# FireflyRenderEngine/GPUPathTracer

Hardware: AMD Instinct MI355X
Metric: Mrays/s (path segments = closest-hit queries, device-counted) at 1080p, 8 bounces, 1024 spp (higher is better)
Workload: dtype f32; 1 GPU; C2 wahoo.obj+cube.obj Cornell box (5184 triangles, 6 planes), 1920x1080, 8 bounces, 1024 spp, camera=inside, trace=bvh, seed 1234; scene=c2, rays_per_frame=11019120206, rays_untraversed=2123366400, rays_cut_last=721266356, primary_hits_kept_between_frames=False, partition=1080-row strips round-robin over 1 rank(s), gather=none

## Files before the change

### gpupathtracer_amd/csrc/ff_api.cpp

```cpp
#include <algorithm>
#include <chrono>
#include <cmath>
#include <cstdio>
#include <cstdlib>
#include <cstring>
#include <new>
#include <vector>

#include <hip/hip_runtime.h>
#include <hip/hip_gl_interop.h>

#include "ff_state.h"

using namespace ff;

namespace {

void free_scene(FfState* s)
{
    s->primary_valid = s->last_key_valid = false;
    if (s->d_geoms) (void)hipFree(s->d_geoms);
    if (s->d_tris) (void)hipFree(s->d_tris);
    if (s->d_normals) (void)hipFree(s->d_normals);
    if (s->d_world_normals) (void)hipFree(s->d_world_normals);
// ... 72 lines not shown
    if (status == FF_OK && ue != hipSuccess) return fail(FF_ERR_HIP, "hipGraphicsUnmapResources failed: %s", hipGetErrorString(ue));
    return status;
}

}

namespace {

int check_params(const FfRenderParams* p)
{
    if (!p) return fail(FF_ERR_INVALID_ARG, "render params are null");
    if (p->width <= 0 || p->height <= 0) return fail(FF_ERR_INVALID_ARG, "image size %dx%d is invalid", p->width, p->height);
    if (p->width > 65535 || p->height > 65535) return fail(FF_ERR_INVALID_ARG, "image size %dx%d exceeds 65535 per side", p->width, p->height);
    if (p->bounces < 1 || p->bounces > 255) return fail(FF_ERR_INVALID_ARG, "bounces must be in 1..255 (got %d)", p->bounces);
    if (p->spp < 1 || p->spp >= (1 << 24)) return fail(FF_ERR_INVALID_ARG, "spp must be in 1..2^24-1 (got %d)", p->spp);
    if (p->trace_mode != FF_TRACE_BRUTE_FORCE && p->trace_mode != FF_TRACE_BVH) return fail(FF_ERR_INVALID_ARG, "unknown trace_mode %d", p->trace_mode);
    if (p->shade_mode != FF_SHADE_NORMAL_DEBUG && p->shade_mode != FF_SHADE_DIFFUSE_PATH && p->shade_mode != FF_SHADE_DIFFUSE_PATH_SMOOTH &&
        p->shade_mode != FF_SHADE_DIFFUSE_PATH_NEE) return fail(FF_ERR_INVALID_ARG, "unknown shade_mode %d", p->shade_mode);
    if (p->grid_mode != FF_GRID_FULL && p->grid_mode != FF_GRID_REFERENCE_FLOOR) return fail(FF_ERR_INVALID_ARG, "unknown grid_mode %d", p->grid_mode);
    if (p->spp_per_launch < 0) return fail(FF_ERR_INVALID_ARG, "spp_per_launch must be >= 0");
    return FF_OK;
}

}

extern "C" int ff_check_render_params(const FfRenderParams* params)
{
    clear_error();
    return check_params(params);
}

namespace ff {

int check_render_call(const FfState* s, const FfCamera* camera, const FfRenderParams* params, const char* who)
{
    if (!s) return fail(FF_ERR_INVALID_ARG, "%s: state is null", who);
    if (!camera) return fail(FF_ERR_INVALID_ARG, "%s: camera is null", who);
    const int st = check_params(params);
    if (st != FF_OK) return st;
    if (!s->has_scene) return fail(FF_ERR_NO_SCENE, "%s: no scene uploaded", who);
    return FF_OK;
}

}

namespace {

int lds_records(const FfState* s) { return s->num_geoms > kMaxLdsRecords ? 0 : s->num_geoms; }

int bvh_block_threads(const FfState* s, int preferred, int stack_levels)
{
    const int sizes[3] = { 1024, 768, 512 };
    for (int b : sizes) {
        if (b > preferred) continue;
        if (bvh_lds_bytes(0, stack_levels, b, lds_records(s)) + (s->use_pool ? pool_lds_bytes(b) : 0) <= (size_t)kLdsBudgetBytes) return b;
    }
    return 0;
}

int finalize_layout(FfState* s)
{
    int nodes4 = 0, depth4 = 0;
    for (size_t i = 0; i < s->slots.size(); ++i) {
        if (s->h_geoms[i].type != FF_GEOM_TRIANGLEMESH || s->slots[i].node4_count == 0) continue;
        nodes4 += s->slots[i].node4_count;
        depth4 = std::max(depth4, s->slots[i].depth4);
    }
    s->num_nodes4 = nodes4;
    s->max_depth4 = depth4;
    s->top_count = s->top_depth = 0;
    if (s->num_geoms > kChunkGeometries) {
        std::vector<BvhNode> top2;
        std::vector<Bvh4Node> top4;
        s->num_scan = s->sw.no_scan_planes ? 0 : count_scan_planes(s->h_geoms, s->num_quads);
        build_geometry_tree(s->h_geoms, top2, s->num_scan);
        s->top_depth = collapse_geometry_tree(top2, top4);
        s->top_count = (int)top4.size();
        if (top4.size() > (size_t)s->num_geoms) return fail(FF_ERR_HIP, "geometry tree of %zu nodes for %d geometries", top4.size(), s->num_geoms);
        FF_HIP(hipMemcpyAsync(s->d_nodes4 + s->node_capacity, top4.data(), top4.size() * sizeof(Bvh4Node), hipMemcpyHostToDevice, s->stream));
        FF_HIP(hipStreamSynchronize(s->stream));
    }
    build_wall_table(s->h_geoms.data(), s->sw.no_wall_table ? 0 : (s->num_geoms > kChunkGeometries ? s->num_scan : s->num_quads), s->walls, !s->sw.no_wall_pairs);
    if (s->num_geoms <= kChunkGeometries) add_mesh_boxes(s->h_geoms.data(), s->num_planes, s->num_geoms, s->walls);
    s->stack_entries = depth4 + 1 + (s->top_depth > 0 ? s->top_depth + 1 : 0);
    if (!s->setup_threshold_forced) {
        int biggest = 1;
        for (size_t i = 0; i < s->slots.size(); ++i) biggest = std::max(biggest, s->slots[i].node4_count);
        s->setup_threshold = std::max(4, std::min(24, (int)std::lround(1.5 * std::log((double)biggest) / std::log(4.0) - 0.7)));
        s->setup_threshold = std::min(32, s->setup_threshold + 2 * s->top_depth);
    }
    s->use_pool = s->sw.pool > 0 && s->num_geoms <= kChunkGeometries && nodes4 > 0;
    constexpr int kPoolStackLevels = 5;
    const int pool_levels = std::min(s->stack_entries, s->sw.pool_stack_levels > 0 ? s->sw.pool_stack_levels : kPoolStackLevels);
    s->scene_block_threads = bvh_block_threads(s, s->block_threads, s->use_pool ? pool_levels : s->stack_entries);
    if (s->use_pool && s->scene_block_threads != 1024) {
        s->use_pool = false;
        s->scene_block_threads = bvh_block_threads(s, s->block_threads, s->stack_entries);
    }
    const int block = s->scene_block_threads > 0 ? s->scene_block_threads : kBlockThreads;
    constexpr int kMinLdsStack = 4;
    const size_t reserve = s->use_pool ? pool_lds_bytes(block) : 0;
    s->stack_lds_levels = s->stack_entries;
    if (s->use_pool) {
        s->stack_lds_levels = pool_levels;
        while (s->stack_lds_levels < s->stack_entries && max_lds_nodes(s->stack_lds_levels + 1, block, lds_records(s), reserve) >= nodes4) ++s->stack_lds_levels;
    } else if (s->scene_block_threads > 0 && !s->sw.no_stack_spill) {
        const int want = nodes4 + s->top_count;
        if (want > max_lds_nodes(s->stack_entries, block, lds_records(s))) {
            int levels = s->stack_entries;
            while (levels > kMinLdsStack && max_lds_nodes(levels, block, lds_records(s)) < want) --levels;
            if (max_lds_nodes(levels, block, lds_records(s)) >= want) s->stack_lds_levels = levels;
        }
    }
    int cap = s->scene_block_threads > 0 ? std::max(0, max_lds_nodes(s->stack_lds_levels, block, lds_records(s), reserve)) : 0;
    if (s->sw.lds_node_cap >= 0) cap = std::min(cap, s->sw.lds_node_cap);
    s->lds_cap = std::min(cap, nodes4 + s->top_count);
    s->top_lds_count = std::min(s->top_count, cap);
    const int mesh_cap = cap - s->top_lds_count;
    constexpr int kSmallTree = 8;
    std::vector<int> share(s->h_geoms.size(), 0);
    int left = mesh_cap, wanting = 0;
    for (size_t i = 0; i < s->h_geoms.size(); ++i) {
        if (s->h_geoms[i].type != FF_GEOM_TRIANGLEMESH || s->slots[i].node4_count == 0) continue;
        share[i] = std::min(std::min(s->slots[i].node4_count, kSmallTree), left);
        left -= share[i];
        wanting += s->slots[i].node4_count - share[i];
    }
    const int pool = left;
    for (size_t i = 0; i < s->h_geoms.size() && wanting > 0; ++i) {
        if (s->h_geoms[i].type != FF_GEOM_TRIANGLEMESH || s->slots[i].node4_count == 0) continue;
        const int want = s->slots[i].node4_count - share[i];
        share[i] += wanting <= pool ? want : (int)((int64_t)pool * want / wanting);
    }
    int next = s->top_lds_count;
    for (size_t i = 0; i < s->h_geoms.size(); ++i) {
        GeomRecord& r = s->h_geoms[i];
        r.node4_first = 0;
        r.lds_nodes = 0;
        r.wmin[3] = 0.0f;
        if (r.type != FF_GEOM_TRIANGLEMESH || s->slots[i].node4_count == 0) continue;
        r.node4_first = s->slots[i].node_first;
        r.lds_nodes = std::min(s->slots[i].node4_count, share[i]);
        std::memcpy(&r.wmin[3], &next, sizeof(int));
        next += r.lds_nodes;
    }
    FF_HIP(hipMemcpyAsync(s->d_geoms, s->h_geoms.data(), s->h_geoms.size() * sizeof(GeomRecord), hipMemcpyHostToDevice, s->stream));
    if (s->d_world_normals) {
        int max_tris = 0;
        for (const GeomRecord& g : s->h_geoms) max_tris = std::max(max_tris, g.type == FF_GEOM_TRIANGLEMESH ? g.tri_count : 0);
        FF_HIP(launch_world_normals(s->d_geoms, s->d_tris, s->num_geoms, max_tris, s->d_world_normals, s->d_world_normals + s->num_tris, s->stream));
    }
    FF_HIP(hipStreamSynchronize(s->stream));
    return FF_OK;
}

int collapse_slot(FfState* s, size_t gi, bool with_info)
{
    FfState::MeshSlot& slot = s->slots[gi];
    if (slot.node_count <= 0) return FF_OK;
    int st = FF_OK;
    if (!slot.parents_linked) {
        st = gpu_link_parents(s->stream, s->d_nodes, slot.node_first, slot.node_count, s->d_parent + slot.node_first);
        if (st != FF_OK) return st;
        slot.parents_linked = true;
    }
    Collapse4Info info;
    st = gpu_collapse_mesh(s->stream, s->scratch, s->d_nodes, slot.node_first, slot.node_count, s->d_parent + slot.node_first, s->d_nodes4, slot.node_first, s->d_role + slot.node_first,
                           with_info ? &info : nullptr);
    if (st != FF_OK) return st;
    if (with_info) {
        if (info.node_count >= (1 << 22)) return fail(FF_ERR_UNSUPPORTED, "a mesh's tree has %d 4-wide nodes; the traversal stack encodes at most %d", info.node_count, (1 << 22) - 1);
        slot.node4_count = info.node_count;
        slot.depth4 = info.depth;
    }
    return FF_OK;
}

int fill_frame_mapping(const FfState* s, KParams& k, const FfCamera* camera, int W, int H, int grid_mode, int strip_rows, int part, int num_parts,
                       int local_rows, int x0, int y0, int win_w, int num_blocks, const char* who)
{
    FfMat4 cm;
    ff_camera_ray_matrix_jittered(camera, s->jitter_x, s->jitter_y, &cm);
    std::memcpy(k.cam_c0, &cm.m[0], 16);
    std::memcpy(k.cam_c1, &cm.m[4], 16);
    std::memcpy(k.cam_c2, &cm.m[8], 16);
    std::memcpy(k.cam_c3, &cm.m[12], 16);
    k.cam_pos[0] = camera->m_position.x;
    k.cam_pos[1] = camera->m_position.y;
    k.cam_pos[2] = camera->m_position.z;
    k.far_clip = camera->m_farClip;
    k.screen_w = camera->m_screenWidth;
    k.screen_h = camera->m_screenHeight;
    k.width = W;
    k.height = H;
    k.xlim = W;
    k.ylim = H;
    if (grid_mode == FF_GRID_REFERENCE_FLOOR) {
        k.xlim = (W / 16) * 16;
        k.ylim = (H / 16) * 16;
    }
    k.strip_rows = strip_rows;
    k.part = part;
    k.num_parts = num_parts;
    k.local_rows = local_rows;
    k.x0 = x0;
    k.y0 = y0;
    k.local_width = win_w;
    k.tiles_per_row = (win_w + 7) / 8;
    const uint64_t tiles = (uint64_t)k.tiles_per_row * (uint64_t)((local_rows + 7) / 8);
    if (tiles * 64 * (uint64_t)(num_blocks + 64) >= (1ull << 31)) return fail(FF_ERR_INVALID_ARG, "%simage too large for the work queue", who);
    k.pix_items = (unsigned)(tiles * 64);
    return FF_OK;
}

void fill_scene(const FfState* s, KParams& k, bool smooth, int lds_block_threads)
{
    k.setup_threshold = s->setup_threshold;
    k.leaf_threshold = s->leaf_threshold;
    k.num_geoms = s->num_geoms;
    k.num_planes = s->num_planes;
    k.num_quads = s->num_quads;
    k.has_specular = s->has_specular ? 1 : 0;
    k.geoms = s->d_geoms;
    k.tris = s->d_tris;
    k.trinormals = smooth ? reinterpret_cast<const float4*>(s->d_normals) : nullptr;
    k.nodes4 = s->d_nodes4;
    k.tri_world_normals = s->d_world_normals;
    k.geom_world_normals = s->d_world_normals ? s->d_world_normals + s->num_tris : nullptr;
    if (s->sw.lds_fill && lds_block_threads > 0) {
        const size_t bytes = bvh_lds_bytes(s->lds_cap, s->stack_lds_levels, lds_block_threads, lds_records(s));
        k.debug_lds_words = (unsigned)std::min<size_t>(s->sw.lds_fill_words, bytes / 4);
        k.debug_lds_pattern = (unsigned)s->sw.lds_fill_pattern;
    }
    k.stack_depth = s->stack_lds_levels;
    k.stack_spill = nullptr;
    k.lds_nodes = s->lds_cap;
    k.top_first = (int)s->node_capacity;
    k.top_lds_first = 0;
    k.top_lds_count = s->top_lds_count;
    k.num_scan = s->num_scan;
    k.walls = s->walls;
}

int attach_stack_spill(FfState* s, KParams& k, int grid, int block_threads)
{
    if (s->stack_lds_levels >= s->stack_entries) return FF_OK;
    const int st = ensure_bytes((void**)&s->d_stack_spill, &s->stack_spill_bytes,
                                (size_t)(s->stack_entries - s->stack_lds_levels) * (size_t)grid * (size_t)block_threads * sizeof(int));
    if (st == FF_OK) k.stack_spill = s->d_stack_spill;
    return st;
}

void size_work_queue(const FfState* s, KParams& k, int grid, int block_threads, int tail_per_wave)
{
    k.queue_counters = std::min(kQueueCountersDefault, grid);
    if (s->sw.queue_counters > 0) k.queue_counters = std::min(std::min(kQueueCounters, grid), s->sw.queue_counters);
    const int waves_per_counter = (grid * (block_threads / 64) + k.queue_counters - 1) / k.queue_counters;
    k.queue_tail_items = (unsigned)(waves_per_counter * (s->sw.queue_tail >= 0 ? s->sw.queue_tail : tail_per_wave));
}

FfState::PrimaryKey primary_key(const KParams& k, bool smooth)
{
    FfState::PrimaryKey key;
    std::memset(&key, 0, sizeof key);
    std::memcpy(key.cam, k.cam_c0, 16 * sizeof(float));
    std::memcpy(key.cam + 16, k.cam_pos, 3 * sizeof(float));
    key.cam[19] = k.far_clip; key.cam[20] = k.screen_w; key.cam[21] = k.screen_h;
    const int dims[12] = { k.width, k.height, k.xlim, k.ylim, k.strip_rows, k.part, k.num_parts, k.local_rows, k.x0, k.y0, k.local_width, smooth ? 1 : 0 };
    std::memcpy(key.dims, dims, sizeof dims);
    key.pix_items = k.pix_items;
    return key;
}

int enqueue_prepass(FfState* s, const KParams& k, float4* hits, unsigned long long* mask_out, int frame_blocks, int grid, int block_threads)
{
    KParams kp = k;
    kp.shade_mode = kShadePrimaryPass;
    kp.primary_hits = hits;
    kp.bounces = 1;
    kp.spp_total = 1;
    kp.block_spp = 1;
    kp.num_blocks = 1;
    kp.block_begin = 0;
    kp.block_end = 1;
    kp.whole_blocks = 1u;
    kp.total_items = kp.pix_items;
    kp.tail_block = -1;
    kp.cull_mask = nullptr;
    kp.cull_mask_out = mask_out;
    kp.frame_blocks = frame_blocks;
    kp.cut_last = 0;
    kp.timeline = nullptr;
    kp.queue_chunk = 32u;
    if (s->sw.queue_chunk > 0) kp.queue_chunk = (unsigned)s->sw.queue_chunk;
    FF_HIP(launch_trace(kp, FF_TRACE_BVH, false, grid, block_threads, s->stream, nullptr, false, true));
    FF_HIP(hipMemsetAsync(s->d_queue, 0, (size_t)k.queue_counters * kQueueStride * sizeof(unsigned), s->stream));
    return FF_OK;
}

}

namespace ff {

int render_enqueue(FfState* s, const FfCamera* camera, const FfRenderParams* prm, int strip_rows, int part, int num_parts, int local_rows,
                   unsigned char* rgb8_dev, float* radiance_dev, int x0, int y0, int win_w)
{
    const int W = prm->width, H = prm->height;
    if (win_w < 0) win_w = W;
    const size_t local_pixels = (size_t)local_rows * (size_t)win_w;
    s->stats = FfStats();
    s->pending = false;
    if (local_pixels == 0) return FF_OK;

    const bool debug = prm->shade_mode == FF_SHADE_NORMAL_DEBUG;
    const bool env = s->env_set && !debug;
    if (env && prm->shade_mode == FF_SHADE_DIFFUSE_PATH_SMOOTH)
        return fail(FF_ERR_UNSUPPORTED, "FF_SHADE_DIFFUSE_PATH_SMOOTH does not render under an environment light (ff_set_environment); "
                    "clear it or use FF_SHADE_DIFFUSE_PATH / FF_SHADE_DIFFUSE_PATH_NEE");
    const bool tex = s->tex_bound > 0 && !debug;
    if (tex && prm->shade_mode == FF_SHADE_DIFFUSE_PATH_SMOOTH)
        return fail(FF_ERR_UNSUPPORTED, "FF_SHADE_DIFFUSE_PATH_SMOOTH does not render albedo textures (ff_set_albedo_texture); "
                    "unbind them or use FF_SHADE_DIFFUSE_PATH / FF_SHADE_DIFFUSE_PATH_NEE");
    const bool glossy = s->glossy_applied > 0 && !debug;
    if (glossy && prm->shade_mode == FF_SHADE_DIFFUSE_PATH_SMOOTH)
// ... 139 lines not shown
        if (pst != FF_OK) return pst;
        k.park = s->d_park;
    }
    if (prm->trace_mode == FF_TRACE_BVH) {
        const int st = attach_stack_spill(s, k, grid, block_threads);
        if (st != FF_OK) return st;
    }

    {
        const int samples_per_item = std::max(1, std::min(k.block_spp, k.spp_total));
        k.queue_chunk = samples_per_item >= 64 ? (num_parts > 1 ? 32u : 64u) : (unsigned)std::min(32, std::max(4, 64 / samples_per_item));
        if (s->sw.queue_chunk > 0) k.queue_chunk = (unsigned)s->sw.queue_chunk;
        size_work_queue(s, k, grid, block_threads, samples_per_item >= 16 && !cull ? 64 : 8);
    }
    hipStream_t st = s->stream;
    if (prm->grid_mode == FF_GRID_REFERENCE_FLOOR) {
        if (rgb8_dev) FF_HIP(hipMemsetAsync(rgb8_dev, 0, local_pixels * 3, st));
        if (radiance_dev) FF_HIP(hipMemsetAsync(radiance_dev, 0, local_pixels * 3 * sizeof(float), st));
    }
    FF_HIP(hipMemsetAsync(s->d_counters, 0, (size_t)(1 + k.queue_counters) * kQueueStride * sizeof(unsigned), st));
    FF_HIP(hipEventRecord(s->ev_begin, st));
    k.tail_block = -1;
    const int last_launch_blocks = num_blocks - (launches - 1) * blocks_per_launch;
    const bool short_frame = num_parts == 1 && !s->tail_forced && num_blocks <= 8;
    const double blocks_per_lane = (double)k.pix_items * (double)last_launch_blocks / ((double)grid * (double)block_threads);
    const int tail_blocks_wanted = s->sw.tail_blocks > 0 ? s->sw.tail_blocks : (num_parts > 1 && blocks_per_lane < 24.0 ? 2 : 1);
    const int tail_blocks = std::max(1, std::min(std::min(tail_blocks_wanted, 3), last_launch_blocks - 1));
    const int tail_n = spp - (num_blocks - tail_blocks) * block_spp;
    const int tail_step = short_frame ? std::max(4, (tail_n + 3) / 4) : std::max(s->tail_group_spp * (block_spp / 64), (tail_n + 15) / 16);
    const bool tail_wanted = !debug && prm->trace_mode == FF_TRACE_BVH && s->tail_group_spp > 0 && tail_step < tail_n &&
                             (short_frame || ((num_parts > 1 || s->tail_forced) && last_launch_blocks >= s->tail_min_blocks));
    const size_t tail_bytes = (size_t)k.pix_items * (size_t)tail_n * sizeof(float4);
    const size_t tail_cap = short_frame ? std::min<size_t>(4ull << 30, s->device_mem_bytes / 50) : (16ull << 30);
    const bool tail_mode = tail_wanted && tail_bytes <= tail_cap;
    if (!tail_mode && s->d_tail_samples && s->tail_samples_bytes > (256ull << 20)) {
        (void)hipFree(s->d_tail_samples);
        s->d_tail_samples = nullptr;
        s->tail_samples_bytes = 0;
    }
    s->pending_flags = (tail_mode ? FF_STATS_TAIL_ITEMS : 0u) | (tail_wanted && !tail_mode ? FF_STATS_TAIL_SKIPPED_TOO_LARGE : 0u);
    if (tail_mode) {
        int tst = ensure_bytes((void**)&s->d_tail_samples, &s->tail_samples_bytes, tail_bytes);
        if (tst != FF_OK) return tst;
        k.tail_samples = s->d_tail_samples;
        k.tail_samples_in_block = tail_n;
        int g = 0;
        k.tail_start[0] = 0;
        while (k.tail_start[g] < tail_n && g < 16) { k.tail_start[g + 1] = std::min(tail_n, k.tail_start[g] + tail_step); ++g; }
        k.tail_groups = g;
    }
    cull = cull && num_blocks - (tail_mode ? tail_blocks : 0) > 0 && !debug;
    const bool exact_cull = reuse && !s->sw.no_primary_cull && num_blocks - (tail_mode ? tail_blocks : 0) > 0;
    const bool kept = reuse && hits_kept && (!(cull || exact_cull) || s->primary_has_mask) && start_kept;
    s->pending_mask_reused = s->pending_mask_built = false;
    if (cull || exact_cull) {
        const size_t mask_bytes = ((size_t)k.pix_items / 64 + 2) * sizeof(unsigned long long);
        if (!kept) {
            const int mst = ensure_bytes((void**)&s->d_cull_mask, &s->cull_mask_bytes, mask_bytes);
            if (mst != FF_OK) return mst;
            if (cull) FF_HIP(launch_cull_mask(k, s->d_cull_mask, st));
            else FF_HIP(hipMemsetAsync(s->d_cull_mask, 0, mask_bytes, st));
            s->pending_mask_built = true;
            if (!reuse) s->primary_has_mask = false;
        } else {
            s->pending_mask_reused = true;
        }
        k.cull_mask = s->d_cull_mask;
        s->pending_culled_rays_per_pixel = (unsigned)(spp - (tail_mode ? tail_n : 0));
    }
    if (reuse && kept) k.primary_hits = s->d_primary_cache;
    k.start_records = use_start ? s->d_start_records : nullptr;
    k.start_bounces = bounces;
    if (reuse && !kept) {
        const int pst = enqueue_prepass(s, k, s->d_primary_cache, exact_cull ? s->d_cull_mask : nullptr, num_blocks, grid, block_threads);
        if (pst != FF_OK) return pst;
        k.primary_hits = s->d_primary_cache;
        s->primary_key = key;
        s->primary_valid = true;
        s->primary_has_mask = cull || exact_cull;
        s->primary_has_start = use_start;
        s->start_bounces = bounces;
        s->start_shade = prm->shade_mode;
    }
    for (int l = 0; l < launches; ++l) {
        k.block_begin = l * blocks_per_launch;
        k.block_end = std::min(num_blocks, (l + 1) * blocks_per_launch);
        k.whole_blocks = (unsigned)(k.block_end - k.block_begin);
        k.total_items = k.pix_items * k.whole_blocks;
        if (tail_mode && l == launches - 1) {
            const unsigned groups = (unsigned)k.tail_groups;
            k.tail_block = num_blocks - tail_blocks;
            k.whole_blocks = (unsigned)(k.block_end - tail_blocks - k.block_begin);
            k.tail_first_item = k.pix_items * k.whole_blocks;
            k.total_items = k.tail_first_item + k.pix_items * groups;
        }
        if (l > 0) FF_HIP(hipMemsetAsync(s->d_queue, 0, (size_t)k.queue_counters * kQueueStride * sizeof(unsigned), st));
        FF_HIP(launch_trace(k, prm->trace_mode, s->collect_stats, grid, block_threads, st, &s->last_kernel_name, pool, false, use_start,
                            !s->sw.no_world_normals));
    }
    FF_HIP(launch_combine(k, st));
    FF_HIP(hipEventRecord(s->ev_end, st));
    FF_HIP(hipMemcpyAsync(s->h_counters, s->d_counters, kCounterWords * sizeof(unsigned long long), hipMemcpyDeviceToHost, st));
    if (k.timeline) {
        const size_t rows = (size_t)s->num_cus * 2 * (kBlockThreads / 64);
        s->h_timeline_rows.resize(rows * kTimelineBuckets);
        FF_HIP(hipMemcpyAsync(s->h_timeline_rows.data(), s->d_timeline, rows * kTimelineBuckets * sizeof(unsigned), hipMemcpyDeviceToHost, st));
    }
    s->pending = true;
    s->pending_launches = launches;
    return FF_OK;
}

int frame_primary_hits(FfState* s, const FfCamera* camera, const FfRenderParams* params, PrimaryHits* out)
{
    const int W = params->width, H = params->height;
    KParams k;
    std::memset(&k, 0, sizeof k);
    int st = fill_frame_mapping(s, k, camera, W, H, params->grid_mode, H, 0, 1, H, 0, 0, W, 1, "ff_gbuffer: ");
    if (st != FF_OK) return st;
    const size_t hits_bytes = (size_t)3 * (size_t)k.pix_items * sizeof(float4);
    bool kept = false;
    for (int smooth = 0; smooth < 2 && !kept; ++smooth) {
        const FfState::PrimaryKey key = primary_key(k, smooth != 0);
        kept = s->primary_valid && s->primary_cache_bytes >= hits_bytes && std::memcmp(&key, &s->primary_key, sizeof key) == 0;
    }
    *out = { s->d_primary_cache, !kept, k.pix_items, k.tiles_per_row, k.xlim, k.ylim };
    if (kept) return FF_OK;
    st = ensure_bytes((void**)&s->d_gb_hits, &s->gb_hits_bytes, hits_bytes);
    if (st != FF_OK) return st;
    out->hits = s->d_gb_hits;
    const int block_threads = s->scene_block_threads;
    const int grid = (int)std::max<uint64_t>(1, std::min<uint64_t>((uint64_t)s->num_cus, ((uint64_t)k.pix_items + (uint64_t)block_threads - 1) / (uint64_t)block_threads));
    fill_scene(s, k, false, block_threads);
    st = attach_stack_spill(s, k, grid, block_threads);
    if (st != FF_OK) return st;
    k.reuse_quorum = s->sw.reuse_quorum;
    k.queue = s->d_queue;
    k.counters = s->d_counters;
    k.timeline_ticks = 1;
    size_work_queue(s, k, grid, block_threads, 8);
    FF_HIP(hipMemsetAsync(s->d_counters, 0, (size_t)(1 + k.queue_counters) * kQueueStride * sizeof(unsigned), s->stream));
    return enqueue_prepass(s, k, s->d_gb_hits, nullptr, 1, grid, block_threads);
}

int render_finish(FfState* s)
{
    if (!s->pending) return FF_OK;
    s->pending = false;
    FF_HIP(hipStreamSynchronize(s->stream));
    float ms = 0.f;
    FF_HIP(hipEventElapsedTime(&ms, s->ev_begin, s->ev_end));
    unsigned long long c[32];
    std::memcpy(c, s->h_counters, sizeof c);
    std::memcpy(s->raw_counters, c, sizeof c);
    if (c[0] != 0)
        return fail(FF_ERR_HIP, "the traversal loop guard cut %llu queries short (a malformed or absurdly deep tree): the frame is not valid", c[0]);
    s->stats.rays_traced = 0;
    for (int j = 0; j < kRaySlots; ++j) s->stats.rays_traced += s->h_counters[kRaySlotStride * (kRaySlotFirst + j)];
    s->stats.rays_answered = 0;
    {
        unsigned long long culled = 0;
        for (int j = 0; j < kRaySlots; ++j) culled += s->h_counters[kCulledPixelsWord + kRaySlotStride * j];
        if (s->pending_mask_reused) culled = s->primary_culled_pixels;
        else if (s->pending_mask_built) s->primary_culled_pixels = culled;
        s->stats.rays_answered += culled * s->pending_culled_rays_per_pixel;
    }
    for (int j = 0; j < kRaySlots; ++j) s->stats.rays_answered += s->h_counters[kAnsweredWord + kRaySlotStride * j];
    s->stats.rays_cut_short = 0;
    for (int j = 0; j < kRaySlots; ++j) s->stats.rays_cut_short += s->h_counters[kCutShortWord + kRaySlotStride * j];
    s->raw_counters[0] = s->stats.rays_traced;
    s->stats.nodes_visited = c[1];
    s->stats.tris_tested = c[2];
    s->stats.planes_tested = c[3];
    s->stats.kernel_ms = ms;
    s->stats.kernel_launches = (uint32_t)s->pending_launches;
    s->stats.flags = s->pending_flags;
    s->stats.scene_bytes_nodes = (uint64_t)s->num_nodes4 * sizeof(Bvh4Node);
    s->stats.scene_bytes_tris = s->num_tris * sizeof(TriRecord);
    return FF_OK;
}

}

namespace {

int render_local(FfState* s, const FfCamera* camera, const FfRenderParams* prm, int strip_rows, int part, int num_parts, int local_rows,
                 unsigned char* rgb8_dev, float* radiance_dev, int x0 = 0, int y0 = 0, int win_w = -1)
{
    const int st = render_enqueue(s, camera, prm, strip_rows, part, num_parts, local_rows, rgb8_dev, radiance_dev, x0, y0, win_w);
    if (st != FF_OK) return st;
    return render_finish(s);
}

}

extern "C" {

namespace {
void read_switches(FfState* s)
{
    FfState::Switches w;
    w.no_last_bounce_cut = std::getenv("FF_NO_LAST_BOUNCE_CUT") != nullptr;
    w.no_primary_cull = std::getenv("FF_NO_PRIMARY_CULL") != nullptr;
    w.no_primary_reuse = std::getenv("FF_NO_PRIMARY_REUSE") != nullptr;
    w.no_primary_cache = std::getenv("FF_NO_PRIMARY_CACHE") != nullptr;
    w.no_start_records = std::getenv("FF_NO_START_RECORDS") != nullptr;
    w.no_world_normals = std::getenv("FF_NO_WORLD_NORMALS") != nullptr;
    if (const char* e = std::getenv("FF_TAIL_BLOCKS")) w.tail_blocks = std::max(1, std::min(3, std::atoi(e)));
    if (const char* e = std::getenv("FF_REUSE_MIN_SPP")) w.reuse_min_spp = std::max(1, std::atoi(e));
    if (const char* e = std::getenv("FF_REUSE_QUORUM")) w.reuse_quorum = std::max(1, std::min(65, std::atoi(e)));
    if (const char* e = std::getenv("FF_QUEUE_CHUNK")) w.queue_chunk = std::max(1, std::min(4096, std::atoi(e)));
    if (const char* e = std::getenv("FF_QUEUE_COUNTERS")) w.queue_counters = std::max(1, std::min(kQueueCounters, std::atoi(e)));
    w.no_wall_table = std::getenv("FF_NO_WALL_TABLE") != nullptr;
    w.no_wall_pairs = std::getenv("FF_NO_WALL_PAIRS") != nullptr;
    w.no_stack_spill = std::getenv("FF_NO_STACK_SPILL") != nullptr;
    w.no_scan_planes = std::getenv("FF_NO_SCAN_PLANES") != nullptr;
    if (const char* e = std::getenv("FF_DEBUG_LDS_FILL")) w.lds_fill = std::sscanf(e, "%lu,%lx", &w.lds_fill_words, &w.lds_fill_pattern) == 2;
    if (const char* e = std::getenv("FF_POOL")) w.pool = std::atoi(e) != 0 ? 1 : 0;
    if (const char* e = std::getenv("FF_POOL_QUORUM")) w.pool_quorum = std::max(1, std::min(64, std::atoi(e)));
    if (const char* e = std::getenv("FF_POOL_QUORUM_MIN")) w.pool_quorum_min = std::max(1, std::min(64, std::atoi(e)));
    if (const char* e = std::getenv("FF_POOL_REFILL")) w.pool_refill = std::max(1, std::min(64, std::atoi(e)));
    if (const char* e = std::getenv("FF_POOL_SLICE")) w.pool_slice = std::max(1, std::min(64, std::atoi(e)));
    if (const char* e = std::getenv("FF_POOL_BATCH_MIN")) w.pool_batch_min = std::max(1, std::min(1024, std::atoi(e)));
    if (const char* e = std::getenv("FF_DEBUG_LDS_NODE_CAP")) w.lds_node_cap = std::max(0, std::atoi(e));
    if (const char* e = std::getenv("FF_QUEUE_TAIL")) w.queue_tail = std::max(0, std::min(4096, std::atoi(e)));
    if (const char* e = std::getenv("FF_POOL_LEAVE")) w.pool_leave = std::max(0, std::min(64, std::atoi(e)));
    if (const char* e = std::getenv("FF_POOL_STACK_LEVELS")) w.pool_stack_levels = std::max(1, std::min(64, std::atoi(e)));
    s->sw = w;
}
}

int ff_debug_reload_switches(FfState* s)
{
    clear_error();
    if (!s) return fail(FF_ERR_INVALID_ARG, "ff_debug_reload_switches: state is null");
    read_switches(s);
    s->primary_valid = s->last_key_valid = false;
    return FF_OK;
}

int ff_create(FfState** out_state, int device_id)
{
    clear_error();
    if (!out_state) return fail(FF_ERR_INVALID_ARG, "ff_create: out_state is null");
    *out_state = nullptr;
    int count = 0;
    hipError_t e = hipGetDeviceCount(&count);
    if (e != hipSuccess || count <= 0) return fail(FF_ERR_NO_DEVICE, "ff_create: no HIP device (%s)", hipGetErrorString(e));
    if (device_id < 0 || device_id >= count) return fail(FF_ERR_INVALID_ARG, "ff_create: device %d out of range (0..%d)", device_id, count - 1);
    FF_HIP(hipSetDevice(device_id));
    hipDeviceProp_t prop;
    FF_HIP(hipGetDeviceProperties(&prop, device_id));
    FfState* s = new (std::nothrow) FfState();
    if (!s) return fail(FF_ERR_OOM, "ff_create: out of host memory");
    s->device = device_id;
    s->num_cus = prop.multiProcessorCount > 0 ? prop.multiProcessorCount : 256;
    s->device_mem_bytes = prop.totalGlobalMem;
    if (const char* bt = std::getenv("FF_BLOCK_THREADS")) {
        const int v = std::atoi(bt);
        if (v == 512 || v == 768 || v == 1024) {
            s->block_threads = v;
        }
    }
    read_switches(s);
    if (const char* e = std::getenv("FF_DEBUG_FAIL_ALLOC")) s->debug_fail_alloc = std::atoi(e);
    if (const char* e = std::getenv("FF_DEBUG_TIMELINE_US")) s->timeline_bucket_us = std::max(0, std::atoi(e));
    if (const char* e = std::getenv("FF_TAIL_MIN_BLOCKS")) s->tail_min_blocks = std::max(1, std::atoi(e));
    if (const char* e = std::getenv("FF_TAIL_GROUP")) {
        s->tail_group_spp = std::max(0, std::min(64, std::atoi(e)));
        s->tail_forced = true;
    }
    if (const char* e = std::getenv("FF_SETUP_THRESHOLD")) {
        s->setup_threshold = std::max(0, std::min(1 << 14, std::atoi(e)));
        s->setup_threshold_forced = true;
    }
    if (const char* e = std::getenv("FF_LEAF_THRESHOLD")) s->leaf_threshold = std::max(1, std::min(64, std::atoi(e)));
    hipError_t pe = prepare_kernels();
    if (pe != hipSuccess) {
        delete s;
        return fail(FF_ERR_HIP, "ff_create: kernel preparation failed: %s (is this a gfx950 device?)", hipGetErrorString(pe));
    }
    if (hipMalloc((void**)&s->d_counters, (size_t)(1 + kQueueCounters) * kQueueStride * sizeof(unsigned)) != hipSuccess ||
        hipHostMalloc((void**)&s->h_counters, kCounterWords * sizeof(unsigned long long), hipHostMallocDefault) != hipSuccess ||
        hipEventCreate(&s->ev_begin) != hipSuccess || hipEventCreate(&s->ev_end) != hipSuccess) {
        ff_destroy(s);
        return fail(FF_ERR_HIP, "ff_create: allocating work buffers failed");
    }
    s->d_queue = reinterpret_cast<unsigned*>(s->d_counters) + kQueueStride;
    *out_state = s;
    return FF_OK;
// ... 833 lines not shown
            mean_dev = s->d_mean;
        }
    }
    st = progressive_frame(s, camera, params, frame_index, rgb8_dev, mean_dev);
    if (st != FF_OK) return st;
    if (rgb8 && !rgb8_on_device) FF_HIP(hipMemcpy(rgb8, rgb8_dev, pixels * 3, hipMemcpyDeviceToHost));
    if (radiance && !radiance_on_device) FF_HIP(hipMemcpy(radiance, mean_dev, pixels * 3 * sizeof(float), hipMemcpyDeviceToHost));
    s->stats.total_ms = std::chrono::duration<double, std::milli>(std::chrono::steady_clock::now() - t0).count();
    return FF_OK;
}

int ff_render_to_pbo_progressive(FfState* s, const FfCamera* camera, const FfRenderParams* params, int frame_index)
{
    clear_error();
    const auto t0 = std::chrono::steady_clock::now();
    if (s && !s->pbo_resource) return fail(FF_ERR_GL_UNAVAILABLE, "ff_render_to_pbo_progressive: no pixel buffer registered");
    int st = check_render_call(s, camera, params, "ff_render_to_pbo_progressive");
    if (st != FF_OK) return st;
    if (params->width != s->pbo_width || params->height != s->pbo_height)
        return fail(FF_ERR_INVALID_ARG, "ff_render_to_pbo_progressive: params are %dx%d but the registered buffer is %dx%d", params->width, params->height,
                    s->pbo_width, s->pbo_height);
    FF_HIP(hipSetDevice(s->device));
    void* dptr = nullptr;
    st = map_pbo(s, (size_t)params->width * (size_t)params->height * 3, &dptr);
    if (st == FF_OK) st = unmap_pbo(s, progressive_frame(s, camera, params, frame_index, (unsigned char*)dptr, nullptr));
    s->stats.total_ms = std::chrono::duration<double, std::milli>(std::chrono::steady_clock::now() - t0).count();
    return st;
}


int ff_set_pixel_jitter(FfState* s, float jx, float jy)
{
    clear_error();
    if (!s) return fail(FF_ERR_INVALID_ARG, "ff_set_pixel_jitter: state is null");
    if (!(jx >= 0.f && jx < 1.f && jy >= 0.f && jy < 1.f))
        return fail(FF_ERR_INVALID_ARG, "ff_set_pixel_jitter: the jitter must be finite and in [0, 1) (got %g %g)", (double)jx, (double)jy);
    s->jitter_x = jx;
    s->jitter_y = jy;
    return FF_OK;
}


int ff_set_collect_stats(FfState* s, int on)
{
    clear_error();
    if (!s) return fail(FF_ERR_INVALID_ARG, "ff_set_collect_stats: state is null");
    s->collect_stats = on != 0;
    return FF_OK;
}

int ff_debug_timeline(FfState* s, unsigned* out1024, int* bucket_us)
{
    clear_error();
    if (!s || !out1024 || !bucket_us) return fail(FF_ERR_INVALID_ARG, "ff_debug_timeline: null argument");
    std::memset(s->h_timeline, 0, sizeof s->h_timeline);
    for (size_t i = 0; i < s->h_timeline_rows.size(); ++i) s->h_timeline[i % kTimelineBuckets] += s->h_timeline_rows[i];
    std::memcpy(out1024, s->h_timeline, sizeof s->h_timeline);
    *bucket_us = s->timeline_bucket_us;
    return FF_OK;
}

int ff_debug_counters(FfState* s, unsigned long long* out32)
{
    clear_error();
    if (!s || !out32) return fail(FF_ERR_INVALID_ARG, "ff_debug_counters: null argument");
    std::memcpy(out32, s->raw_counters, sizeof s->raw_counters);
    return FF_OK;
}

int ff_debug_check_ieee(FfState* s, unsigned long long* out_mismatches2)
{
    clear_error();
    if (!s || !out_mismatches2) return fail(FF_ERR_INVALID_ARG, "ff_debug_check_ieee: null argument");
    FF_HIP(hipSetDevice(s->device));
    FF_HIP(hipMemsetAsync(s->d_counters, 0, 2 * sizeof(unsigned long long), s->stream));
    FF_HIP(launch_ieee_check(s->d_counters, s->stream));
    FF_HIP(hipMemcpyAsync(out_mismatches2, s->d_counters, 2 * sizeof(unsigned long long), hipMemcpyDeviceToHost, s->stream));
    FF_HIP(hipStreamSynchronize(s->stream));
    return FF_OK;
}

const char* ff_debug_kernel_name(FfState* s) { return s && s->last_kernel_name ? s->last_kernel_name : ""; }

int ff_stats(FfState* s, FfStats* out)
{
    clear_error();
    if (!s || !out) return fail(FF_ERR_INVALID_ARG, "ff_stats: null argument");
    *out = s->stats;
    return FF_OK;
}

}
```

### gpupathtracer_amd/csrc/ff_internal.h

```cpp
#pragma once

#include <cstdarg>
#include <cstdint>
#include <string>
#include <vector>

#include "../../include/firefly/ff_api.h"
#include "ff_texture.h"

namespace ff {

int fail(int status, const char* fmt, ...) __attribute__((format(printf, 2, 3)));
void clear_error();


struct TriRecord {
    float v0[3];
    int32_t orig_index;
    float e1[3];
    float cull_margin;
    float e2[3];
    int32_t pad1;
};
static_assert(sizeof(TriRecord) == 48, "48-byte triangle record");

struct TriNormals {
    float n0[3], pad0;
    float n1[3], pad1;
    float n2[3], pad2;
};
static_assert(sizeof(TriNormals) == 48, "48-byte vertex-normal record");

struct BvhNode {
    float lmin[3];
    int32_t left;
    float lmax[3];
    int32_t right;
    float rmin[3];
    int32_t pad0;
    float rmax[3];
    int32_t pad1;
};
static_assert(sizeof(BvhNode) == 64, "64-byte BVH node");

struct Bvh4Node {
    float mn[3][4];
    float mx[3][4];
    int32_t link[4];
};
static_assert(sizeof(Bvh4Node) == 112, "112-byte 4-wide BVH node");
constexpr int32_t kEmptyLink = 0x7fffffff;

struct GeomRecord {
    float inv_c0[4], inv_c1[4], inv_c2[4], inv_c3[4];
    float mod_c0[4], mod_c1[4], mod_c2[4], mod_c3[4];
    float nrm_c0[4], nrm_c1[4], nrm_c2[4];
    float plane_n[4];
    float albedo[4];
    float emission[4];
    float wmin[4], wmax[4];
    int32_t type;
    int32_t bxdf_type;
    int32_t tri_first;
    int32_t tri_count;
    int32_t bvh_root;
    int32_t orig_index;
    int32_t node4_first;
    int32_t lds_nodes;
};
static_assert(sizeof(GeomRecord) == 16 * 16 + 32, "GeomRecord layout");

constexpr int kMaxWalls = 16;
struct Wall {
    float c;
    float cu, hu;
    float cv, hv;
    int geom;
    int hi_geom1;
    float hi_c;
};
static_assert(sizeof(Wall) == 32, "32-byte wall");
struct WallTable {
    int count[3];
    unsigned mask;
    float margin_s;
    float graze;
    int num_boxes;
    int pad;
    Wall w[kMaxWalls];
    struct MeshBox {
        float mn[3];
        int geom;
        float mx[3];
        int pad;
    } box[32];
};

void build_wall_table(const struct GeomRecord* geoms, int limit, WallTable& out, bool pairing = true);
void add_mesh_boxes(const struct GeomRecord* geoms, int first, int n, WallTable& out);

struct CompiledScene {
    std::vector<GeomRecord> geoms;
    std::vector<TriRecord> tris;
    std::vector<TriNormals> normals;
    std::vector<TriUVs> uvs;
    std::vector<BvhNode> nodes;
    int max_depth = 0;
    uint64_t total_tris = 0;
};

struct BvhBuildParams {
    int max_leaf_tris = 2;
    int device_leaf_tris = 2;
    int max_depth = 30;
    int bins = 64;
    float c_trav = 1.2f;
    int opt_passes = 1;
    int opt_max_tris = 1 << 18;
};

BvhBuildParams default_bvh_params();

int build_mesh_bvh(const FfTriangle* triangles, int count, const BvhBuildParams& params, std::vector<BvhNode>& nodes,
                   std::vector<TriRecord>& tris, int* out_depth, std::vector<TriNormals>* normals = nullptr, std::vector<TriUVs>* uvs = nullptr);

int compile_scene(const FfGeometry* geoms, int n, const BvhBuildParams& params, CompiledScene& out, bool build_bvh = true);

int build_geometry_tree(const std::vector<GeomRecord>& geoms, std::vector<BvhNode>& nodes, int first);
constexpr int kMaxScanPlanes = 8;
int count_scan_planes(const std::vector<GeomRecord>& geoms, int num_quads);

constexpr int32_t kGeomLeafBit = 0x40000000;
int collapse_geometry_tree(const std::vector<BvhNode>& binary, std::vector<Bvh4Node>& out);

void set_world_box(GeomRecord& r, const float omn[3], const float omx[3]);

}
```

### gpupathtracer_amd/csrc/ff_k_traverse.h

```cpp
#pragma once
#include "ff_k_lds.h"

namespace ff {
namespace {


constexpr int kLoopGuard = 1 << 16;
constexpr float kRel = 1.0e-4f, kAbs = 1.0e-4f;

struct Pending {
    float dist;
    int geom;
    int rec;
};

struct Segment {
    BestId best;
    Pending pend;
    unsigned meshes;
    int cur, sp, mesh;
    int tl_sp;
    int node_base;
    int lds_first, lds_count;
    int bnx, bny, bnz;
// ... 120 lines not shown
        const float sdist = tt * wlen * __builtin_amdgcn_rcpf(len);
        if (tt > 0.0f && offer(sdist, g, -1, S.pend, S.best)) {
            HitPoint H;
            resolve_pending(L, tris, wr, S.pend, S.best, H);
            offer(sdist, g, -1, S.pend, S.best);
        }
        return;
    }
    const float4 c0 = lds_geom4(L, g, 0), c1 = lds_geom4(L, g, 1), c2 = lds_geom4(L, g, 2), c3 = lds_geom4(L, g, 3);
    const float4 pn = lds_geom4(L, g, 11);
    const float ox = __builtin_fmaf(c0.x, wr.ox, __builtin_fmaf(c1.x, wr.oy, __builtin_fmaf(c2.x, wr.oz, c3.x)));
    const float oy = __builtin_fmaf(c0.y, wr.ox, __builtin_fmaf(c1.y, wr.oy, __builtin_fmaf(c2.y, wr.oz, c3.y)));
    const float oz = __builtin_fmaf(c0.z, wr.ox, __builtin_fmaf(c1.z, wr.oy, __builtin_fmaf(c2.z, wr.oz, c3.z)));
    const float ux = __builtin_fmaf(c0.x, wr.dx, __builtin_fmaf(c1.x, wr.dy, c2.x * wr.dz));
    const float uy = __builtin_fmaf(c0.y, wr.dx, __builtin_fmaf(c1.y, wr.dy, c2.y * wr.dz));
    const float uz = __builtin_fmaf(c0.z, wr.dx, __builtin_fmaf(c1.z, wr.dy, c2.z * wr.dz));
    const float nx = pn.x, ny = pn.y, nz = pn.z;
    const float dn = __builtin_fmaf(nx, ux, __builtin_fmaf(ny, uy, nz * uz));
    const float num = -__builtin_fmaf(nx, ox, __builtin_fmaf(ny, oy, nz * oz));
    const float len2 = __builtin_fmaf(ux, ux, __builtin_fmaf(uy, uy, uz * uz));
    const float q = dn * dn, qlim = 1.0e-14f * len2;
    const float ta = num * __builtin_amdgcn_rcpf(dn);
    const float Pxa = __builtin_fmaf(ta, ux, ox), Pya = __builtin_fmaf(ta, uy, oy);
    const float omag = fabsf(ox) + fabsf(oy) + fabsf(oz);
    const float delta = 1.0e-5f * (1.0f + omag) * __builtin_fmaf(fabsf(ux) + fabsf(uy), fabsf(__builtin_amdgcn_rcpf(dn)), 1.0f);
    const float ex = fabsf(Pxa), ey = fabsf(Pya);
    const bool front_sure = ta > 0.0f && fabsf(num) > 1.0e-5f * omag * (fabsf(nx) + fabsf(ny) + fabsf(nz));
    bool hit = ex <= 0.5f - delta && ey <= 0.5f - delta && front_sure && q >= qlim * 1.01f;
    float dist = ta * wlen;
    if (!hit && ex <= 0.5f + delta && ey <= 0.5f + delta && q >= qlim * 0.99f && (front_sure || fabsf(num) <= 1.0e-5f * omag * (fabsf(nx) + fabsf(ny) + fabsf(nz)))) {
        if (STATS) cnt.plane_exact += 1;
        Ray osr;
        float len;
        object_space_ray_lds(L, g, wr, osr, len);
        const float tt = plane_t(nx, ny, nz, osr);
        hit = tt > 0.0f;
        dist = tt * wlen * __builtin_amdgcn_rcpf(len);
    }
    if (hit && offer(dist, g, -1, S.pend, S.best)) {
        HitPoint H;
        resolve_pending(L, tris, wr, S.pend, S.best, H);
        offer(dist, g, -1, S.pend, S.best);
    }
}

__device__ __forceinline__ void wall_test(const Wall& w, float ixk, float oxk, float ou, float du, float ov, float dv, float dl, float tt, bool steep,
                                          float wlen, float& best_d, int& best_g, bool& tie, unsigned& slow)
{
    const float t = __builtin_fmaf(w.c, ixk, oxk);
    const float pu = __builtin_fmaf(t, du, ou), pv = __builtin_fmaf(t, dv, ov);
    const float m = fmaxf(fabsf(pu - w.cu) - w.hu, fabsf(pv - w.cv) - w.hv);
    const bool hit = m <= -dl && t > tt && steep;
    const bool miss = m > dl || t < -tt;
    slow |= (!hit && !miss) ? 1u << w.geom : 0u;
    const float d = t * wlen;
    const bool nearer = hit && best_d > __builtin_fmaf(d, 1.0f + kRel, kAbs);
    const bool farther = d > __builtin_fmaf(best_d, 1.0f + kRel, kAbs);
    tie = tie || (hit && !nearer && !farther);
    best_d = nearer ? d : best_d;
    best_g = nearer ? w.geom : best_g;
}

__device__ __forceinline__ void wall_test_pair(const Wall& w, float ixk, float oxk, float ou, float du, float ov, float dv, float dl, float tt, bool steep,
                                               float wlen, float& best_d, int& best_g, bool& tie, unsigned& slow)
{
    const float tlo = __builtin_fmaf(w.c, ixk, oxk), thi = __builtin_fmaf(w.hi_c, ixk, oxk);
    const bool up = ixk > 0.0f;
    const float t = up ? thi : tlo, tother = up ? tlo : thi;
    const int g = up ? w.hi_geom1 - 1 : w.geom, gother = up ? w.geom : w.hi_geom1 - 1;
    slow |= !(tother < -tt) ? 1u << gother : 0u;
    const float pu = __builtin_fmaf(t, du, ou), pv = __builtin_fmaf(t, dv, ov);
    const float m = fmaxf(fabsf(pu - w.cu) - w.hu, fabsf(pv - w.cv) - w.hv);
    const bool hit = m <= -dl && t > tt && steep;
    const bool miss = m > dl || t < -tt;
    slow |= (!hit && !miss) ? 1u << g : 0u;
    const float d = t * wlen;
    const bool nearer = hit && best_d > __builtin_fmaf(d, 1.0f + kRel, kAbs);
    const bool farther = d > __builtin_fmaf(best_d, 1.0f + kRel, kAbs);
    tie = tie || (hit && !nearer && !farther);
    best_d = nearer ? d : best_d;
    best_g = nearer ? g : best_g;
}

template <bool STATS>
__device__ __forceinline__ void screen_walls(const WallTable& W, const Ray& wr, const WorldSlab& ws, float wlen, Segment& S, unsigned& slow, Counters& cnt)
{
    const int nx = W.count[0], ny = nx + W.count[1], nz = ny + W.count[2];
    if (nz == 0) return;
    if (STATS) { cnt.planes += (unsigned)nz; probe_round(cnt.wall_rounds); }
    const float D = 2.0e-5f * ((fabsf(wr.ox) + fabsf(wr.oy)) + (fabsf(wr.oz) + W.margin_s));
    const float th = 0.05f * D;
    const float ax = fabsf(wr.dx), ay = fabsf(wr.dy), az = fabsf(wr.dz);
    const float aix = fabsf(ws.ix), aiy = fabsf(ws.iy), aiz = fabsf(ws.iz);
    const float gmin = W.graze * wlen;
    float best_d = kInf;
    int best_g = -1;
    bool tie = false;
    Wall cur = W.w[0];
    int i = 0;
    {
        const float dl = D * __builtin_fmaf(fmaxf(ay, az), aix, 1.0f), tt = th * aix;
        const bool steep = ax >= gmin;
        for (; i < nx; ++i) {
            const Wall nxt = W.w[min(i + 1, kMaxWalls - 1)];
            if (cur.hi_geom1) wall_test_pair(cur, ws.ix, ws.ox, wr.oy, wr.dy, wr.oz, wr.dz, dl, tt, steep, wlen, best_d, best_g, tie, slow);
            else wall_test(cur, ws.ix, ws.ox, wr.oy, wr.dy, wr.oz, wr.dz, dl, tt, steep, wlen, best_d, best_g, tie, slow);
            cur = nxt;
        }
    }
    {
        const float dl = D * __builtin_fmaf(fmaxf(az, ax), aiy, 1.0f), tt = th * aiy;
        const bool steep = ay >= gmin;
        for (; i < ny; ++i) {
            const Wall nxt = W.w[min(i + 1, kMaxWalls - 1)];
            if (cur.hi_geom1) wall_test_pair(cur, ws.iy, ws.oy, wr.oz, wr.dz, wr.ox, wr.dx, dl, tt, steep, wlen, best_d, best_g, tie, slow);
            else wall_test(cur, ws.iy, ws.oy, wr.oz, wr.dz, wr.ox, wr.dx, dl, tt, steep, wlen, best_d, best_g, tie, slow);
            cur = nxt;
        }
    }
    {
        const float dl = D * __builtin_fmaf(fmaxf(ax, ay), aiz, 1.0f), tt = th * aiz;
        const bool steep = az >= gmin;
        for (; i < nz; ++i) {
            const Wall nxt = W.w[min(i + 1, kMaxWalls - 1)];
            if (cur.hi_geom1) wall_test_pair(cur, ws.iz, ws.oz, wr.ox, wr.dx, wr.oy, wr.dy, dl, tt, steep, wlen, best_d, best_g, tie, slow);
            else wall_test(cur, ws.iz, ws.oz, wr.ox, wr.dx, wr.oy, wr.dy, dl, tt, steep, wlen, best_d, best_g, tie, slow);
            cur = nxt;
        }
    }
    if (tie) {
        slow |= W.mask;
    } else if (best_g >= 0) {
        S.pend.dist = best_d;
        S.pend.geom = best_g;
        S.pend.rec = -1;
    }
}

__device__ __forceinline__ unsigned holds(const Segment& S)
{
    return (S.pend.geom >= 0 ? 1u << (S.pend.geom & 31) : 0u) | (S.best.geom >= 0 ? 1u << (S.best.geom & 31) : 0u);
}

template <bool STATS, class LDS>
__device__ __forceinline__ bool scan_records(const LDS& L, const WallTable& W, const GeomRecord* __restrict__ geoms, int num_geoms, int num_planes,
                                           const TriRecord* __restrict__ tris, const Ray& wr, Segment& S, Counters& cnt, bool cut, unsigned emitters)
{
    const int prim_end = num_planes;
    const float wlen = __builtin_amdgcn_rcpf(inv_length(wr));

    unsigned long long tb0 = 0, tb1 = 0, tb2 = 0;
    if (STATS) tb0 = __builtin_amdgcn_s_memtime();
    const WorldSlab ws = make_world_slab(wr);
    unsigned quads = 0u;
    screen_walls<STATS>(W, wr, ws, wlen, S, quads, cnt);
    for (int g = 0; g < prim_end; ++g) {
        if ((W.mask >> g) & 1u) continue;
        const float4 bmin = lds_geom4(L, g, 14), bmax = lds_geom4(L, g, 15);
        if (slab_may_hit(bmin.x, bmin.y, bmin.z, bmax.x, bmax.y, bmax.z, ws, kInf)) quads |= 1u << g;
    }
    if (STATS) tb1 = __builtin_amdgcn_s_memtime();
    for (int guard = 0; __ballot(quads != 0u) != 0ull && guard < 32; ++guard) {
        if (quads == 0u) continue;
        const int g = __ffs((int)quads) - 1;
        quads &= quads - 1u;
        screen_analytic<STATS>(L, g, tris, wr, wlen, S, cnt);
    }

    if (STATS) tb2 = __builtin_amdgcn_s_memtime();
    S.meshes = 0u;
    const float limit = fminf(S.best.dist, S.pend.dist);
    {
        typedef unsigned box_words __attribute__((ext_vector_type(8)));
        static_assert(sizeof(WallTable::MeshBox) == 32, "one box, one load");
        box_words cur = *reinterpret_cast<const box_words*>(&W.box[0]);
        for (int i = 0; i < W.num_boxes; ++i) {
            const box_words nxt = *reinterpret_cast<const box_words*>(&W.box[min(i + 1, 31)]);
            S.meshes |= slab_may_hit(__uint_as_float(cur.s0), __uint_as_float(cur.s1), __uint_as_float(cur.s2), __uint_as_float(cur.s4), __uint_as_float(cur.s5),
                                     __uint_as_float(cur.s6), ws, limit) ? 1u << cur.s3 : 0u;
            cur = nxt;
        }
    }
    const bool over = cut && (holds(S) & emitters) == 0u;
    if (over) S.meshes = 0u;
    if (STATS && S.meshes == 0u) cnt.no_mesh += 1;
    if (STATS) {
        const unsigned long long tb3 = __builtin_amdgcn_s_memtime();
        if ((threadIdx.x & 63) == __ffsll((long long)__ballot(true)) - 1) { cnt.t_b1 += tb1 - tb0; cnt.t_b2 += tb2 - tb1; cnt.t_b3 += tb3 - tb2; }
    }
    return over;
}

template <class LDS>
__device__ __forceinline__ void enter_top(const LDS& L, const Ray& wr, Segment& S);

template <bool STATS, class LDS>
__device__ __forceinline__ void scan_walls(const LDS& L, const WallTable& W, const TriRecord* __restrict__ tris, const Ray& wr, Segment& S, Counters& cnt)
{
    const float wlen = __builtin_amdgcn_rcpf(inv_length(wr));
    const WorldSlab ws = make_world_slab(wr);
    unsigned prims = 0u;
    screen_walls<STATS>(W, wr, ws, wlen, S, prims, cnt);
    for (int g = 0; g < L.num_scan; ++g) {
        if ((W.mask >> g) & 1u) continue;
        const float4 bmin = lds_geom4(L, g, 14), bmax = lds_geom4(L, g, 15);
        if (slab_may_hit(bmin.x, bmin.y, bmin.z, bmax.x, bmax.y, bmax.z, ws, kInf)) prims |= 1u << g;
    }
    for (int guard = 0; __ballot(prims != 0u) != 0ull && guard < 8; ++guard) {
        if (prims == 0u) continue;
        const int g = __ffs((int)prims) - 1;
        prims &= prims - 1u;
        screen_analytic<STATS>(L, g, tris, wr, wlen, S, cnt);
    }
}

template <bool STATS, class LDS>
__device__ __forceinline__ bool begin_segment(const LDS& L, const WallTable& W, const GeomRecord* __restrict__ geoms, int num_geoms, int num_planes,
                                              const TriRecord* __restrict__ tris, const Ray& wr, Segment& S, Counters& cnt, bool cut = false,
                                              unsigned emitters = 0u)
{
    S.best.dist = kInf;
    S.best.geom = -1;
    S.best.rec = -1;
    S.pend.dist = kInf;
    S.pend.geom = -1;
    S.pend.rec = -1;
    S.cur = kDone;
    S.sp = 0;
    S.tl_sp = 0;
    S.mesh = -1;
    S.resume = 0;
    if constexpr (LDS::big) {
        S.meshes = 0u;
        if (L.num_scan > 0) scan_walls<STATS>(L, W, tris, wr, S, cnt);
        const bool over = cut && (holds(S) & emitters) == 0u;
        if (over) return true;
        enter_top(L, wr, S);
        S.cur = 0;
        return false;
    }
    return scan_records<STATS>(L, W, geoms, num_geoms, num_planes, tris, wr, S, cnt, cut, emitters);
}

__device__ __forceinline__ void refresh_tbound(Segment& S)
{
    S.tbound = (fminf(S.best.dist, S.pend.dist) * 1.001f + 1.0e-3f) * S.scale * 1.00001f;
}

#define FF_PIN4(q) asm volatile("" : "+v"((q).x), "+v"((q).y), "+v"((q).z), "+v"((q).w))

__device__ __forceinline__ int select_slot(const uint4 q, int c)
{
    const unsigned m0 = (unsigned)((c << 31) >> 31), m1 = (unsigned)((c << 30) >> 31);
    const unsigned lo = (q.y & m0) | (q.x & ~m0), hi = (q.w & m0) | (q.z & ~m0);
    return (int)((hi & m1) | (lo & ~m1));
}

template <class LDS>
__device__ __forceinline__ void pop_entry(const LDS& L, const uint4* __restrict__ nodes4, Segment& S, int e)
{
    if (e >= 0 && (e & kPackedEntry) != 0) {
        const int node = (e >> 8) & 0x3FFFFF;
        uint4 lk;
        if ((unsigned)node < (unsigned)S.lds_count) {
            lk = ff_smem[S.lds_first + node + 6 * L.node_cap];
            FF_PIN4(lk);
        } else {
            lk = *reinterpret_cast<const uint4*>(reinterpret_cast<const char*>(nodes4) + ((unsigned)(S.node_base + node) * (unsigned)(kNodeVec4 * 16) + 96u));
            FF_PIN4(lk);
        }
        S.cur = select_slot(lk, (e >> 2) & 3);
        const int rest = (e & 3) == 2 ? select_slot(lk, (e >> 4) & 3)
                                      : ((e & ~0xFF) | (((e >> 4) & 0xF) << 2) | 2);
        stack_push(L, S.sp - 1, rest);
    } else {
        S.cur = e;
        --S.sp;
    }
}

template <class LDS>
__device__ __forceinline__ void pop_subtree(const LDS& L, const uint4* __restrict__ nodes4, Segment& S)
{
    if (S.sp == (LDS::big ? S.tl_sp : 0)) {
        S.cur = LDS::big && S.mesh >= 0 ? kMeshDone : kDone;
        return;
    }
    pop_entry(L, nodes4, S, stack_pop(L, S.sp - 1));
}

template <class LDS>
__device__ __forceinline__ void set_box_planes(const LDS& L, Segment& S)
{
    const int q = L.node_cap * 16;
    S.bnx = S.ix < 0.0f ? 3 * q : 0;
    S.bny = S.iy < 0.0f ? 4 * q : q;
    S.bnz = S.iz < 0.0f ? 5 * q : 2 * q;
    S.bfx = 3 * q - S.bnx;
    S.bfy = 5 * q - S.bny;
    S.bfz = 7 * q - S.bnz;
}

template <class LDS>
__device__ __forceinline__ void enter_mesh(const LDS& L, int g, const Ray& wr, Segment& S)
{
    const int4 tree = lds_geom_i4(L, g, 17);
    if (tree.x < 0) return;
    float len;
    object_space_ray_lds(L, g, wr, S.osr, len);
    S.ix = safe_rcp(S.osr.dx);
    S.iy = safe_rcp(S.osr.dy);
    S.iz = safe_rcp(S.osr.dz);
    S.ox = -S.osr.ox * S.ix;
    S.oy = -S.osr.oy * S.iy;
    S.oz = -S.osr.oz * S.iz;
    set_box_planes(L, S);
    S.scale = len * inv_length(wr);
    refresh_tbound(S);
    S.mesh = g;
    S.node_base = tree.z;
    S.lds_count = tree.w;
    S.lds_first = __float_as_int(lds_geom4(L, g, 14).w);
    S.cur = 0;
    if constexpr (!LDS::big) S.sp = 0;
// ... 341 lines not shown
```

### gpupathtracer_amd/csrc/ff_kernels.h

```cpp
#pragma once

#include <hip/hip_runtime.h>

#include "ff_internal.h"

namespace ff {

constexpr int kBlockThreads = 512;
constexpr int kBlockThreadsMax = 1024;
constexpr int kLdsBudgetBytes = 160 * 1024;
constexpr int kMaxLdsRecords = 128;
constexpr int kChunkGeometries = 32;
constexpr int kBruteBatchTris = 1024;

struct KParams {
    float cam_c0[4], cam_c1[4], cam_c2[4], cam_c3[4];
    float cam_pos[3];
    float far_clip;
    float screen_w, screen_h;
    int width, height;
    int xlim, ylim;
    int strip_rows, part, num_parts, local_rows;
    int x0, y0, local_width;
    unsigned whole_blocks;
    unsigned total_items;
    unsigned queue_chunk;
    unsigned queue_tail_items;
    unsigned pix_items;
    int tiles_per_row;
    int bounces, spp_total, block_spp, block_begin, block_end, num_blocks;
    unsigned key;
    int shade_mode;
    int setup_threshold, leaf_threshold;
    int num_geoms;
    int num_planes;
    int num_quads;
    int has_specular;
    const GeomRecord* geoms;
    const TriRecord* tris;
    const float4* trinormals;
    int num_scan;
    const Bvh4Node* nodes4;
    int top_first, top_lds_first, top_lds_count;
    int lds_nodes;
    int stack_depth;
    int* stack_spill;
    float4* blocksums;
    unsigned char* rgb8;
    float* radiance;
    unsigned* queue;
    int queue_counters;
    int tail_block;
    int tail_groups;
    int tail_start[17];
    int tail_samples_in_block;
    unsigned tail_first_item;
    float4* tail_samples;
    unsigned long long* counters;
    unsigned debug_lds_words, debug_lds_pattern;
    const unsigned long long* cull_mask;
    unsigned long long* cull_mask_out;
    int frame_blocks;
    float4* primary_hits;
    int reuse_quorum;
    unsigned emitter_mask;
    int cut_last;
    float scene_min[3], scene_max[3];
    WallTable walls;
    float4* park;
    int pool_quorum, pool_quorum_min, pool_refill, pool_slice, pool_leave, pool_batch_min;
    unsigned* timeline;
    unsigned timeline_ticks;
    float4* start_records;
    int start_bounces;
    const float4* tri_world_normals;
    const float4* geom_world_normals;
};
constexpr int kRaySlots = 30, kRaySlotFirst = 2, kRaySlotStride = 16;
constexpr int kAnsweredWord = kRaySlotStride * kRaySlotFirst + 1;
constexpr int kCutShortWord = kRaySlotStride * kRaySlotFirst + 3;
constexpr int kCulledPixelsWord = kRaySlotStride * kRaySlotFirst + 2;
constexpr int kCounterWords = 512;
constexpr int kTimelineBuckets = 1024;
constexpr int kQueueCounters = 64;
constexpr int kQueueCountersDefault = 16;
constexpr int kQueueStride = 1024;
constexpr int kShadePrimaryPass = 100;
constexpr int kQueueStripe = 64;
constexpr int kQueueTailWord = 64;

struct RayBatchParams {
    const FfRay* rays;
    FfIntersect* out;
    int n;
    int num_geoms;
    int num_planes;
    int num_quads;
    const GeomRecord* geoms;
    const TriRecord* tris;
    const Bvh4Node* nodes4;
    int top_first, top_lds_first, top_lds_count;
    int lds_nodes;
    int stack_depth;
    int* stack_spill;
    int num_scan;
    WallTable walls;
    unsigned long long* guard_hits;
};

constexpr unsigned kNeeKeySelect = 0x6A09E667u;
constexpr unsigned kNeeKeyPoint = 0xBB67AE85u;
struct NeeParams {
    KParams k;
    const float4* lights;
    int num_lights;
    const float* light_pdf;
    unsigned items;
    const float4* env_texels;
    const float2* env_alias;
    const float* env_z;
    int env_w, env_h;
    float env_rotation;
    float p_env;
    float p_area;
    const TexBinding* tex_bind;
    const TexDesc* tex_desc;
    const TriUVs* uvs;
    const float* glossy_alpha;
    int cam_active, cam_box;
    float cam_lens_radius, cam_focus;
    float cam_fwd[3], cam_right[3], cam_up[3];
};
constexpr unsigned kEnvKeyChoose = 0x3C6EF372u;
constexpr unsigned kCameraKeyPixel = 0xA54FF53Au;
constexpr unsigned kCameraKeyLens = 0x510E527Fu;

size_t bvh_lds_bytes(int lds_nodes, int stack_depth, int block_threads, int num_geoms);
int max_lds_nodes(int stack_depth, int block_threads, int num_geoms, size_t reserve = 0);
size_t pool_lds_bytes(int block_threads);

hipError_t launch_trace(const KParams& p, int trace_mode, bool collect_stats, int grid_blocks, int block_threads, hipStream_t stream,
                        const char** kernel_name = nullptr, bool pool = false, bool prepass = false, bool start = false, bool world_normals = false);
hipError_t launch_world_normals(const GeomRecord* geoms, const TriRecord* tris, int num_geoms, int max_tri_count, float4* tri_out, float4* geom_out,
                                hipStream_t stream);
hipError_t launch_combine(const KParams& p, hipStream_t stream);
hipError_t launch_cull_mask(const KParams& p, unsigned long long* mask, hipStream_t stream);
hipError_t launch_accumulate(float* sum, const float* frame, float* mean, unsigned char* rgb8, size_t values, int first_frame, float inv_frames,
                             hipStream_t stream);
hipError_t launch_ray_batch(const RayBatchParams& p, int trace_mode, hipStream_t stream);
hipError_t launch_ieee_check(unsigned long long* mismatches2, hipStream_t stream);
hipError_t launch_deinterleave(const void* src, void* dst, int width, int height, int strip_rows, int num_parts, int elem_bytes,
                               hipStream_t stream);
hipError_t launch_unpack_strips(const void* src, unsigned char* rgb8, float* radiance, int width, int height, int strip_rows, int num_parts,
                                hipStream_t stream);
hipError_t launch_nee(const NeeParams& np, int trace_mode, bool env, bool tex, bool glossy, int grid_blocks, hipStream_t stream, const char** kernel_name);
hipError_t prepare_kernels();

}
```

### gpupathtracer_amd/csrc/ff_kernels.hip

```cpp
#include "ff_k_traverse.h"
#include "ff_k_shade.h"

namespace ff {
namespace {


template <bool STATS, int BLOCK, bool EXTRAS, int BIG = 0, bool PREPASS = false, bool START = false, bool WN = false>
__global__ __launch_bounds__(BLOCK) void trace_bvh_kernel(const KParams p)
{
    static_assert(!START || (!EXTRAS && BIG == 0 && !PREPASS), "start records: the diffuse small-scene kernel only");
    static_assert(!WN || (!EXTRAS && BIG == 0 && !PREPASS), "normal tables: the diffuse small-scene kernels only");
    const int tid = threadIdx.x;
    const int lane = tid & (kWave - 1);
    const LdsT<BIG> L = make_lds<BIG>(p.lds_nodes, p.stack_depth, BLOCK, tid, EXTRAS ? p.num_quads : 0x7fffffff, EXTRAS ? p.trinormals : nullptr,
                                      p.geoms, p.top_first, p.top_lds_first, p.top_lds_count, BIG ? p.num_scan : 0, p.stack_spill);
    const uint4* nodes4 = reinterpret_cast<const uint4*>(p.nodes4);
    if (p.debug_lds_words != 0u) {
        for (unsigned i = tid; i < p.debug_lds_words; i += BLOCK) reinterpret_cast<unsigned*>(ff_smem)[i] = p.debug_lds_pattern;
        __syncthreads();
    }
    stage_scene(L, nodes4, p.geoms, p.num_geoms, p.num_planes, tid, BLOCK);
    if constexpr (WN) {
        for (int g = tid; g < p.num_planes; g += BLOCK) reinterpret_cast<float4*>(ff_smem)[L.geom_base + g * kGeomVec4 + kGeomWorldNormalVec4] = p.geom_world_normals[g];
        __syncthreads();
    }

    Counters cnt = {};
    Path P;
    init_path(P);
    WaveQueue Q = make_wave_queue(p);
    Segment S;
    S.best = { kInf, -1, -1 };
    S.pend = { kInf, -1, -1 };
    S.meshes = 0u;
    S.cur = kDone; S.sp = 0; S.mesh = -1; S.resume = 0;
    S.osr = { 0.f, 0.f, 0.f, 0.f, 0.f, 1.f };
    S.ix = S.iy = S.iz = S.ox = S.oy = S.oz = 0.f;
    S.scale = 1.f;
    S.tbound = 0.f;
    S.node_base = 0; S.lds_first = 0; S.lds_count = 0; S.tl_sp = 0;
    S.bnx = S.bny = S.bnz = S.bfx = S.bfy = S.bfz = 0;
    bool active = false, exhausted = false, inflight = false;
    const bool reuse = START || (!PREPASS && p.primary_hits != nullptr);
    auto stored_hit = [&](int k) { return p.primary_hits + (size_t)k * p.pix_items + ((unsigned)P.item & kItemPixelMask); };
    unsigned long long tphase[5] = { 0, 0, 0, 0, 0 };
    const unsigned long long wave_t0 = STATS ? wall_clock64() : 0ull;
    unsigned long long epoch = 0ull;
    if (STATS && p.timeline) {
        if (lane == 0) {
            const unsigned long long seen = atomicCAS(&p.counters[27], 0ull, wave_t0);
            epoch = seen ? seen : wave_t0;
        }
        epoch = __shfl(epoch, 0);
    }
    unsigned* const tl_row = STATS && p.timeline ? p.timeline + (size_t)(blockIdx.x * (BLOCK / kWave) + tid / kWave) * kTimelineBuckets : nullptr;
    int tl_bucket = 0;
    unsigned tl_count = 0u;
    for (;;) {
        unsigned long long t0 = 0, t1 = 0, t2 = 0, t3 = 0, t4 = 0;
        if (STATS) t0 = __builtin_amdgcn_s_memtime();
        const bool setup = !inflight || segment_done(S);
        if (STATS && p.timeline) {
            const int finished = __popcll(__ballot(setup && inflight));
            if (finished) {
                const unsigned long long now = wall_clock64();
                const unsigned long long bb = now > epoch ? (now - epoch) / p.timeline_ticks : 0ull;
                const int b = bb < (unsigned long long)kTimelineBuckets ? (int)bb : kTimelineBuckets - 1;
                if (b != tl_bucket) {
                    if (lane == 0 && tl_count) tl_row[tl_bucket] += tl_count;
                    tl_bucket = b;
                    tl_count = 0u;
                }
                tl_count += (unsigned)finished;
            }
        }
        Best best;
        bool hit = false;
        bool shade_now = setup && inflight;
        if (shade_now) {
            finish_segment<WN>(L, p.tris, P.ray, S, best, p.tri_world_normals);
            hit = best.geom >= 0;
        }
        if (STATS) t1 = __builtin_amdgcn_s_memtime();
        if constexpr (START) {
            bool from_rec = setup && !inflight && active && P.b == 0;
            bool goes_on = false;
            MaterialRef M;
            M.global = nullptr;
            M.geom_base = L.geom_base;
            M.g = 0;
            if (shade_now) {
                M.g = best.geom;
                const int r = settle_hit<false, false, WN>(p, best, hit, M, P);
                inflight = false;
// ... 4 lines not shown
            float4 q0 = make_float4(0.f, 0.f, 0.f, 0.f), q1 = q0;
            if (from_rec) {
                const float4* rec = p.start_records + ((unsigned)P.item & kItemPixelMask);
                q0 = rec[0];
                q1 = rec[p.pix_items];
                cnt.rays += 1;
                goes_on = true;
            }
            {
                const unsigned reused_now = (unsigned)__popcll(__ballot(from_rec));
                cnt.reused += reused_now;
                if (STATS && p.timeline) tl_count += reused_now;
            }
            if (goes_on) scatter_start<WN>(p, best, M, P, from_rec, q0, q1);
        } else {
            bool from_cache = setup && !inflight && active && P.b == 0 && reuse;
            bool settle_now = shade_now, goes_on = false;
            for (;;) {
                if (from_cache) {
                    const float4 c0 = *stored_hit(0), c1 = *stored_hit(1), c2 = *stored_hit(2);
                    best.dist = c0.x; best.px = c0.y; best.py = c0.z; best.pz = c0.w;
                    best.cx = c1.x; best.cy = c1.y; best.cz = c1.z;
                    best.geom = __float_as_int(c1.w);
                    best.rec = __float_as_int(c2.x);
                    hit = best.geom >= 0;
                    if constexpr (WN) {
                        float4 n = make_float4(0.f, 0.f, 1.f, 0.f);
                        if (hit) {
                            if (best.rec >= 0) n = p.tri_world_normals[best.rec];
                            else n = lds_geom4(L, best.geom, kGeomWorldNormalVec4);
                        }
                        best.cx = n.x; best.cy = n.y; best.cz = n.z;
                    }
                    cnt.rays += 1;
                    settle_now = true;
                }
                {
                    const unsigned reused_now = (unsigned)__popcll(__ballot(from_cache));
                    cnt.reused += reused_now;
                    if (STATS && p.timeline) tl_count += reused_now;
                }
                if (__ballot(settle_now) == 0ull) break;
                bool waiting = false;
                if (settle_now) {
                    MaterialRef M;
                    M.global = BIG == 2 ? p.geoms + (hit ? best.geom : 0) : nullptr;
                    M.geom_base = L.geom_base;
                    M.g = best.geom;
                    const int r = settle_hit<EXTRAS, PREPASS, WN>(p, best, hit, M, P);
                    inflight = false;
                    active = r != kPixelDone;
                    goes_on = r == kGoesOn;
                    waiting = r == kNewSample && reuse;
                }
                settle_now = false;
                from_cache = waiting && __popcll(__ballot(waiting)) >= p.reuse_quorum;
            }
            if (goes_on) {
                MaterialRef M;
                M.global = BIG == 2 ? p.geoms + best.geom : nullptr;
                M.geom_base = L.geom_base;
                M.g = best.geom;
                scatter<EXTRAS, WN>(p, best, M, P);
            }
        }
        if (STATS) t2 = __builtin_amdgcn_s_memtime();
        {
            const bool need = setup && !active && !exhausted;
            if (__ballot(need) != 0ull) {
                const unsigned rays_before = cnt.rays;
                const bool got = acquire_pixel<START>(p, lane, P, Q, need, cnt.rays, &cnt.reused);
                if (STATS && p.timeline) tl_count += (unsigned)wave_sum((unsigned long long)(cnt.rays - rays_before));
                if (need) {
                    active = got;
                    exhausted = !got;
                    if (STATS && exhausted) atomicMax(&p.counters[23], ~(unsigned long long)wall_clock64());
                }
            }
        }
        if (STATS) t3 = __builtin_amdgcn_s_memtime();
        bool over = false;
        if (setup && active && !(P.b == 0 && reuse)) {
            if (STATS) probe_round(cnt.segment_rounds);
            over = begin_segment<STATS>(L, p.walls, p.geoms, p.num_geoms, p.num_planes, p.tris, P.ray, S, cnt, p.cut_last != 0 && P.b == p.bounces - 1, p.emitter_mask);
            cnt.rays += 1;
            inflight = true;
        }
        cnt.cut += (unsigned)__popcll(__ballot(over));
        if (STATS) t4 = __builtin_amdgcn_s_memtime();
        if (__ballot(inflight || (active && P.b == 0 && reuse)) == 0ull) break;
        if (inflight) traverse_budget<STATS>(L, p.tris, nodes4, P.ray, S, cnt, p.setup_threshold, p.leaf_threshold, p.num_planes);
        if (STATS) {
            const unsigned long long t5 = __builtin_amdgcn_s_memtime();
            tphase[0] += t1 - t0; tphase[1] += t2 - t1; tphase[2] += t3 - t2; tphase[3] += t4 - t3; tphase[4] += t5 - t4;
        }
    }
    if (STATS && p.timeline && lane == 0 && tl_count) tl_row[tl_bucket] += tl_count;
    if (STATS && lane == 0) {
        atomicAdd(&p.counters[4], tphase[0]);
        atomicAdd(&p.counters[5], tphase[1]);
        atomicAdd(&p.counters[6], tphase[2]);
        atomicAdd(&p.counters[7], tphase[3]);
        atomicAdd(&p.counters[13], tphase[4]);
        atomicMax(&p.counters[22], tphase[0] + tphase[1] + tphase[2] + tphase[3] + tphase[4]);
        atomicMax(&p.counters[24], ~(unsigned long long)wave_t0);
        atomicMax(&p.counters[25], (unsigned long long)wall_clock64());
    }
    flush_counters(p, lane, cnt, STATS);
}


constexpr int kPoolRing = 2048;
constexpr unsigned kRingEmpty = 0xFFFFu;
constexpr int kPoolSpinLimit = 1 << 20;
constexpr int kPendEmpty = -2;
constexpr int kPendOwner = -3;
constexpr unsigned kJobReturned = 0x80000000u;
constexpr unsigned kJobTie = 0x40000000u;

struct PoolOccupancy {
    unsigned inner_rounds, inner_lanes;
    unsigned leaf_rounds, leaf_lanes;
};

struct PoolRef {
    int job_base;
    int ring_base;
    int ctrl;
};

__device__ __forceinline__ unsigned* pool_u32() { return reinterpret_cast<unsigned*>(ff_smem); }
__device__ __forceinline__ unsigned short* pool_u16() { return reinterpret_cast<unsigned short*>(ff_smem); }

__device__ __forceinline__ void pool_push(const PoolRef& Q, int lane, int slot, bool post)
{
    const unsigned long long m = __ballot(post);
    if (m == 0ull) return;
    __builtin_amdgcn_fence(__ATOMIC_RELEASE, "workgroup");
    const int leader = __ffsll((long long)m) - 1;
    unsigned base = 0u;
    if (lane == leader) base = __hip_atomic_fetch_add(&pool_u32()[Q.ctrl + 1], (unsigned)__popcll(m), __ATOMIC_RELAXED, __HIP_MEMORY_SCOPE_WORKGROUP);
    base = (unsigned)__builtin_amdgcn_readlane((int)base, leader);
    if (post) {
        const unsigned rank = (unsigned)__popcll(m & ((1ull << lane) - 1ull));
        __hip_atomic_store(&pool_u16()[Q.ring_base + (int)((base + rank) & (unsigned)(kPoolRing - 1))], (unsigned short)slot, __ATOMIC_RELAXED, __HIP_MEMORY_SCOPE_WORKGROUP);
    }
}

__device__ __forceinline__ int pool_pop(const PoolRef& Q, int lane, bool want, bool& stuck)
{
    const unsigned long long m = __ballot(want);
    const unsigned asked = (unsigned)__popcll(m);
    unsigned h = 0u, n = 0u;
    if (lane == 0) {
        for (int tries = 0; tries < kPoolSpinLimit; ++tries) {
            h = __hip_atomic_load(&pool_u32()[Q.ctrl], __ATOMIC_RELAXED, __HIP_MEMORY_SCOPE_WORKGROUP);
            const unsigned t = __hip_atomic_load(&pool_u32()[Q.ctrl + 1], __ATOMIC_RELAXED, __HIP_MEMORY_SCOPE_WORKGROUP);
            n = min(asked, t - h);
            if (n == 0u) break;
            unsigned expect = h;
            if (__hip_atomic_compare_exchange_strong(&pool_u32()[Q.ctrl], &expect, h + n, __ATOMIC_RELAXED, __ATOMIC_RELAXED, __HIP_MEMORY_SCOPE_WORKGROUP)) break;
            n = 0u;
        }
    }
    h = (unsigned)__builtin_amdgcn_readfirstlane((int)h);
    n = (unsigned)__builtin_amdgcn_readfirstlane((int)n);
    int slot = -1;
// ... 545 lines not shown
    if (live) {
        const FfRay r = p.rays[i];
        wr.ox = r.m_origin.x; wr.oy = r.m_origin.y; wr.oz = r.m_origin.z;
        wr.dx = r.m_direction.x; wr.dy = r.m_direction.y; wr.dz = r.m_direction.z;
    }
    Best best;
    best.dist = kInf; best.geom = -1; best.rec = -1; best.px = best.py = best.pz = 0.f; best.cx = best.cy = 0.f; best.cz = 1.f;
    Counters cnt = {};
    if (MODE == FF_TRACE_BRUTE_FORCE) closest_hit_brute<false>(p.geoms, p.num_geoms, p.tris, batch, live, wr, best, cnt);
    else if (live) closest_hit_deferred<false>(L, p.walls, p.geoms, p.num_geoms, p.num_planes, p.tris, nodes4, wr, best, cnt);
    if (live && ((cnt.guard_hits >> (threadIdx.x & 63)) & 1ull) != 0ull && p.guard_hits) atomicAdd(p.guard_hits, 1ull);
    if (!live) return;
    FfIntersect out;
    out.m_intersectionPoint.x = 0.f; out.m_intersectionPoint.y = 0.f; out.m_intersectionPoint.z = 0.f;
    out.m_normal.x = 0.f; out.m_normal.y = 0.f; out.m_normal.z = 0.f;
    out.m_t = 0.f;
    out.m_hit = 0;
    out._pad[0] = out._pad[1] = out._pad[2] = 0;
    out.geometryIndex = -1;
    out.triangleIndex = -1;
    if (best.geom >= 0) {
        const GeomRecord& G = p.geoms[best.geom];
        MaterialRef M;
        M.global = &G;
        M.geom_base = L.geom_base;
        M.g = 0;
        float nx, ny, nz;
        world_normal(M, best, true, nx, ny, nz);
        out.m_intersectionPoint.x = best.px; out.m_intersectionPoint.y = best.py; out.m_intersectionPoint.z = best.pz;
        out.m_normal.x = nx; out.m_normal.y = ny; out.m_normal.z = nz;
        out.m_t = best.dist;
        out.m_hit = 1;
        out.geometryIndex = G.orig_index;
        out.triangleIndex = best.rec >= 0 ? p.tris[best.rec].orig_index : -1;
    }
    p.out[i] = out;
}

}
}

#include "ff_k_nee.h"

namespace ff {

#if defined(FF_PROBE) || defined(FF_PROBE_NEE)
namespace {
#ifdef FF_PROBE
template __global__ void FF_PROBE(const KParams);
#else
template __global__ void FF_PROBE_NEE(const NeeParams);
#endif
}
#else
size_t bvh_lds_bytes(int lds_nodes, int stack_depth, int block_threads, int num_geoms)
{
    return (size_t)lds_nodes * sizeof(Bvh4Node) + (size_t)stack_depth * (size_t)block_threads * sizeof(unsigned) +
           (size_t)num_geoms * sizeof(GeomRecord);
}

int max_lds_nodes(int stack_depth, int block_threads, int num_geoms, size_t reserve)
{
    const long avail = (long)kLdsBudgetBytes - (long)reserve - (long)stack_depth * (long)block_threads * (long)sizeof(unsigned) -
                       (long)num_geoms * (long)sizeof(GeomRecord);
    return avail > 0 ? (int)(avail / (long)sizeof(Bvh4Node)) : 0;
}

static int scene_size_class(int num_geoms) { return num_geoms <= kChunkGeometries ? 0 : (num_geoms <= kMaxLdsRecords ? 1 : 2); }

static size_t trace_lds_bytes(bool bvh, int lds_nodes, int stack_depth, int block_threads, int num_geoms, int big)
{
    return bvh ? bvh_lds_bytes(lds_nodes, stack_depth, block_threads, big == 2 ? 0 : num_geoms) : (size_t)kBruteBatchTris * sizeof(TriRecord);
}

static bool needs_extras(const KParams& p) { return p.num_planes > p.num_quads || p.has_specular != 0 || p.trinormals != nullptr; }

template <class K>
static hipError_t allow_full_lds(K* kernel)
{
    return hipFuncSetAttribute(reinterpret_cast<const void*>(kernel), hipFuncAttributeMaxDynamicSharedMemorySize, kLdsBudgetBytes);
}


#define FF_TRACE_BVH_KERNELS_OF(X, B)                                                                                                                \
    X(false, B, false, 0, false, false, false) X(true, B, false, 0, false, false, false) X(false, B, true, 0, false, false, false)                   \
    X(true, B, true, 0, false, false, false) X(false, B, true, 1, false, false, false) X(true, B, true, 1, false, false, false)                      \
    X(false, B, true, 2, false, false, false) X(true, B, true, 2, false, false, false)                                                               \
    X(false, B, true, 0, true, false, false) X(false, B, true, 1, true, false, false) X(false, B, true, 2, true, false, false)                       \
    X(false, B, false, 0, false, true, false) X(true, B, false, 0, false, true, false)                                                               \
    X(false, B, false, 0, false, false, true) X(true, B, false, 0, false, false, true)                                                               \
    X(false, B, false, 0, false, true, true) X(true, B, false, 0, false, true, true)
#define FF_TRACE_BVH_KERNELS(X) FF_TRACE_BVH_KERNELS_OF(X, 512) FF_TRACE_BVH_KERNELS_OF(X, 768) FF_TRACE_BVH_KERNELS_OF(X, 1024)
#define FF_NAME_START_false ""
#define FF_NAME_START_true ", true"
#define FF_RAY_BATCH_KERNELS(X) X(FF_TRACE_BVH, 0) X(FF_TRACE_BVH, 1) X(FF_TRACE_BVH, 2) X(FF_TRACE_BRUTE_FORCE, 0)

#define FF_TRACE_POOL_KERNELS(X) X(false, 1024, false) X(false, 1024, true) X(true, 1024, false) X(true, 1024, true)

#define FF_NEE_KERNELS_OF(X, MODE, BIG)                                                                               \
    X(MODE, BIG, 0, 0, 0, 0, "")           X(MODE, BIG, 1, 0, 0, 0, ", 1")                                            \
    X(MODE, BIG, 0, 1, 0, 0, ", 0, 1")     X(MODE, BIG, 1, 1, 0, 0, ", 1, 1")                                         \
    X(MODE, BIG, 0, 0, 1, 0, ", 0, 0, 1")  X(MODE, BIG, 1, 0, 1, 0, ", 1, 0, 1")                                      \
    X(MODE, BIG, 0, 1, 1, 0, ", 0, 1, 1")  X(MODE, BIG, 1, 1, 1, 0, ", 1, 1, 1")                                      \
    X(MODE, BIG, 0, 0, 0, 1, ", 0, 0, 0, 1") X(MODE, BIG, 1, 0, 0, 1, ", 1, 0, 0, 1")                                 \
    X(MODE, BIG, 0, 1, 0, 1, ", 0, 1, 0, 1") X(MODE, BIG, 1, 1, 0, 1, ", 1, 1, 0, 1")                                 \
    X(MODE, BIG, 0, 0, 1, 1, ", 0, 0, 1, 1") X(MODE, BIG, 1, 0, 1, 1, ", 1, 0, 1, 1")                                 \
    X(MODE, BIG, 0, 1, 1, 1, ", 0, 1, 1, 1") X(MODE, BIG, 1, 1, 1, 1, ", 1, 1, 1, 1")
#define FF_NEE_KERNELS(X) FF_NEE_KERNELS_OF(X, 1, 0) FF_NEE_KERNELS_OF(X, 1, 1) FF_NEE_KERNELS_OF(X, 1, 2) FF_NEE_KERNELS_OF(X, 0, 0)
static_assert(FF_TRACE_BVH == 1 && FF_TRACE_BRUTE_FORCE == 0, "the MODE column and the reported names spell the trace modes as numerals");

hipError_t prepare_kernels()
{
    hipError_t e;
#define FF_X(STATS, B, EXTRAS, BIG, PREPASS, START, WN) \
    if ((e = allow_full_lds(&trace_bvh_kernel<STATS, B, EXTRAS, BIG, PREPASS, START, WN>)) != hipSuccess) return e;
    FF_TRACE_BVH_KERNELS(FF_X)
#undef FF_X
#define FF_X(STATS, B, EXTRAS) \
    if ((e = allow_full_lds(&trace_pool_kernel<STATS, B, EXTRAS>)) != hipSuccess) return e;
    FF_TRACE_POOL_KERNELS(FF_X)
#undef FF_X
#define FF_X(MODE, BIG) \
    if (MODE == FF_TRACE_BVH && (e = allow_full_lds(&ray_batch_kernel<MODE, BIG>)) != hipSuccess) return e;
    FF_RAY_BATCH_KERNELS(FF_X)
#undef FF_X
#define FF_X(MODE, BIG, ENV, TEX, GLOSSY, CAM, TAIL) \
    if (MODE == FF_TRACE_BVH && (e = allow_full_lds(&nee_path_kernel<MODE, BIG, ENV, TEX, GLOSSY, CAM>)) != hipSuccess) return e;
    FF_NEE_KERNELS(FF_X)
#undef FF_X
    return hipSuccess;
}

size_t pool_lds_bytes(int block_threads) { return (size_t)block_threads * 48 + (size_t)kPoolRing * 2 + 128; }

static hipError_t launch_pool(const KParams& p, bool collect_stats, int grid_blocks, int block_threads, hipStream_t stream, const char** kernel_name)
{
    const dim3 grid(grid_blocks), block(block_threads);
    const size_t lds = bvh_lds_bytes(p.lds_nodes, p.stack_depth, block_threads, p.num_geoms) + pool_lds_bytes(block_threads);
    const bool extras = needs_extras(p);
    const char* name = "";
#define FF_X(STATS, B, EXTRAS)                                                                                  \
    if (collect_stats == STATS && block_threads == B && extras == EXTRAS) {                                     \
        hipLaunchKernelGGL((trace_pool_kernel<STATS, B, EXTRAS>), grid, block, lds, stream, p);                 \
        name = "trace_pool_kernel<" #STATS ", " #B ", " #EXTRAS ">";                                            \
    } else
    FF_TRACE_POOL_KERNELS(FF_X) return hipErrorInvalidValue;
#undef FF_X
    if (kernel_name) *kernel_name = name;
    return hipGetLastError();
}

hipError_t launch_trace(const KParams& p, int trace_mode, bool collect_stats, int grid_blocks, int block_threads, hipStream_t stream,
                        const char** kernel_name, bool pool, bool prepass, bool start, bool world_normals)
{
    const dim3 grid(grid_blocks);
    const char* name = "";
    if (!prepass && trace_mode == FF_TRACE_BVH && pool && p.num_geoms <= kChunkGeometries && block_threads == 1024)
        return launch_pool(p, collect_stats, grid_blocks, block_threads, stream, kernel_name);
    if (prepass || trace_mode == FF_TRACE_BVH) {
        const dim3 block(block_threads);
        const int big = scene_size_class(p.num_geoms);
        const size_t lds = trace_lds_bytes(true, p.lds_nodes, p.stack_depth, block_threads, p.num_geoms, big);
        if (!prepass && start && (big != 0 || needs_extras(p) || p.start_records == nullptr)) return hipErrorInvalidValue;
        const int threads = block_threads == 1024 ? 1024 : (block_threads == 768 ? 768 : 512);
        const bool stats = !prepass && collect_stats, extras = prepass || big != 0 || needs_extras(p), from_start = !prepass && start;
        const bool wn = world_normals && !extras && p.shade_mode == FF_SHADE_DIFFUSE_PATH && p.tri_world_normals != nullptr && p.geom_world_normals != nullptr;
#define FF_X(STATS, B, EXTRAS, BIG, PREPASS, START, WN)                                                                                              \
    if (stats == STATS && threads == B && extras == EXTRAS && big == BIG && prepass == PREPASS && from_start == START && wn == WN) {                 \
        hipLaunchKernelGGL((trace_bvh_kernel<STATS, B, EXTRAS, BIG, PREPASS, START, WN>), grid, block, lds, stream, p);                              \
        name = "trace_bvh_kernel<" #STATS ", " #B ", " #EXTRAS ", " #BIG ", " #PREPASS FF_NAME_START_##START ">";                                    \
    } else
        FF_TRACE_BVH_KERNELS(FF_X) return hipErrorInvalidValue;
#undef FF_X
        if (prepass) name = "trace_bvh_kernel<false, B, true, big, true>";
    } else {
        const size_t lds = (size_t)kBruteBatchTris * sizeof(TriRecord);
        const dim3 block(kBlockThreads);
        if (collect_stats) hipLaunchKernelGGL((trace_brute_kernel<true>), grid, block, lds, stream, p);
        else hipLaunchKernelGGL((trace_brute_kernel<false>), grid, block, lds, stream, p);
        name = collect_stats ? "trace_brute_kernel<true>" : "trace_brute_kernel<false>";
    }
    if (kernel_name) *kernel_name = name;
    return hipGetLastError();
}

hipError_t launch_ray_batch(const RayBatchParams& p, int trace_mode, hipStream_t stream)
{
    if (p.n <= 0) return hipSuccess;
    const bool bvh = trace_mode == FF_TRACE_BVH;
    const int mode = bvh ? FF_TRACE_BVH : FF_TRACE_BRUTE_FORCE, big = scene_size_class(p.num_geoms), big_key = bvh ? big : 0;
    const size_t lds = trace_lds_bytes(bvh, p.lds_nodes, p.stack_depth, kBlockThreads, p.num_geoms, big);
    const dim3 grid((p.n + kBlockThreads - 1) / kBlockThreads), block(kBlockThreads);
#define FF_X(MODE, BIG) \
    if (mode == MODE && big_key == BIG) hipLaunchKernelGGL((ray_batch_kernel<MODE, BIG>), grid, block, lds, stream, p); else
    FF_RAY_BATCH_KERNELS(FF_X) return hipErrorInvalidValue;
#undef FF_X
    return hipGetLastError();
}

hipError_t launch_nee(const NeeParams& np, int trace_mode, bool env, bool tex, bool glossy, int grid_blocks, hipStream_t stream, const char** kernel_name)
{
    if (np.items == 0u) return hipSuccess;
    const KParams& p = np.k;
    const bool bvh = trace_mode == FF_TRACE_BVH, cam = np.cam_active != 0;
    const int mode = bvh ? 1 : 0, big = scene_size_class(p.num_geoms), big_key = bvh ? big : 0;
    const size_t lds = trace_lds_bytes(bvh, p.lds_nodes, p.stack_depth, kBlockThreads, p.num_geoms, big);
    const dim3 grid(grid_blocks), block(kBlockThreads);
    const char* name = "";
#define FF_X(MODE, BIG, ENV, TEX, GLOSSY, CAM, TAIL)                                                                  \
    if (mode == MODE && big_key == BIG && env == (ENV != 0) && tex == (TEX != 0) && glossy == (GLOSSY != 0) && cam == (CAM != 0)) { \
        hipLaunchKernelGGL((nee_path_kernel<MODE, BIG, ENV, TEX, GLOSSY, CAM>), grid, block, lds, stream, np);        \
        name = "nee_path_kernel<" #MODE ", " #BIG TAIL ">";                                                           \
    } else
    FF_NEE_KERNELS(FF_X) return hipErrorInvalidValue;
#undef FF_X
    if (kernel_name) *kernel_name = name;
    return hipGetLastError();
}

#endif
}
```

### gpupathtracer_amd/csrc/ff_scene.cpp

```cpp
#include <algorithm>
#include <atomic>
#include <cfloat>
#include <cmath>
#include <cstdio>
#include <cstdlib>
#include <cstring>
#include <limits>
#include <numeric>
#include <queue>
#include <system_error>
#include <thread>

#include "ff_internal.h"
#include "ff_math.h"

namespace ff {

namespace {

struct Box {
    float mn[3], mx[3];
    void reset()
    {
        for (int k = 0; k < 3; ++k) {
// ... 601 lines not shown
        for (int k = 0; k < 3; ++k) { mn[k] = std::min(mn[k], r.wmin[k]); mx[k] = std::max(mx[k], r.wmax[k]); }
    }
    const double scene = box_half_area(mn, mx);
    int n = 0;
    while (n < num_quads && n < kMaxScanPlanes && n + 2 < (int)geoms.size() && scene > 0.0 && box_half_area(geoms[n].wmin, geoms[n].wmax) >= 0.08 * scene) ++n;
    return n;
}

void build_wall_table(const GeomRecord* geoms, int limit, WallTable& out, bool pairing)
{
    std::memset(&out, 0, sizeof out);
    struct Found {
        int axis;
        Wall w;
    };
    std::vector<Found> found;
    float scale_s = 0.f, ratio = 1.f;
    for (int g = 0; g < limit && g < 32 && (int)found.size() < kMaxWalls; ++g) {
        const GeomRecord& r = geoms[g];
        if (r.type != FF_GEOM_PLANE) continue;
        if (!(r.plane_n[0] == 0.f && r.plane_n[1] == 0.f && r.plane_n[2] == 1.f)) continue;
        const float* col[3] = { r.mod_c0, r.mod_c1, r.mod_c2 };
        int dom[3];
        float len[3];
        bool ok = true;
        for (int j = 0; j < 3 && ok; ++j) {
            const float a0 = std::fabs(col[j][0]), a1 = std::fabs(col[j][1]), a2 = std::fabs(col[j][2]);
            dom[j] = a0 >= a1 && a0 >= a2 ? 0 : (a1 >= a2 ? 1 : 2);
            len[j] = std::sqrt(a0 * a0 + a1 * a1 + a2 * a2);
            if (!(len[j] > 1e-20f && len[j] < 1e20f)) ok = false;
            for (int k = 0; k < 3 && ok; ++k)
                if (k != dom[j] && std::fabs(col[j][k]) > 2.0e-7f * len[j]) ok = false;
        }
        if (!ok || dom[0] == dom[1] || dom[0] == dom[2] || dom[1] == dom[2]) continue;
        const float smax = std::max(len[0], std::max(len[1], len[2])), smin = std::min(len[0], std::min(len[1], len[2]));
        if (!(smax <= 16.f * smin)) continue;
        const float* T = r.mod_c3;
        if (!(std::fabs(T[0]) < 1e8f && std::fabs(T[1]) < 1e8f && std::fabs(T[2]) < 1e8f)) continue;
        Found f;
        f.axis = dom[2];
        const int u = (f.axis + 1) % 3, v = (f.axis + 2) % 3;
        const float hu = 0.5f * (dom[0] == u ? len[0] : len[1]), hv = 0.5f * (dom[0] == v ? len[0] : len[1]);
        std::memset(&f.w, 0, sizeof f.w);
        f.w.c = T[f.axis];
        f.w.cu = T[u];
        f.w.hu = hu;
        f.w.cv = T[v];
        f.w.hv = hv;
        f.w.geom = g;
        found.push_back(f);
        ratio = std::max(ratio, smax / smin);
        scale_s = std::max(scale_s, smax + std::fabs(T[0]) + std::fabs(T[1]) + std::fabs(T[2]));
    }
    std::vector<char> used(found.size(), 0);
    int n = 0;
    for (int axis = 0; axis < 3; ++axis)
        for (size_t i = 0; i < found.size(); ++i) {
            if (found[i].axis != axis || used[i]) continue;
            used[i] = 1;
            Wall w = found[i].w;
            out.mask |= 1u << w.geom;
            for (size_t j = i + 1; pairing && j < found.size(); ++j) {
                const Wall& o = found[j].w;
                if (found[j].axis != axis || used[j] || o.c == w.c) continue;
                if (std::memcmp(&o.cu, &w.cu, 4 * sizeof(float)) != 0) continue;
                used[j] = 1;
                out.mask |= 1u << o.geom;
                const Wall& lo = o.c < w.c ? o : w;
                const Wall& hi = o.c < w.c ? w : o;
                Wall both = lo;
                both.hi_geom1 = hi.geom + 1;
                both.hi_c = hi.c;
                w = both;
                break;
            }
            out.w[n++] = w;
            out.count[axis] += 1;
        }
    out.margin_s = ratio * scale_s;
    out.graze = 1.2e-7f * ratio;
    if (ratio > 1.f) {
        out.margin_s += (ratio - 1.f) * 3.f * scale_s;
    }
}

void add_mesh_boxes(const GeomRecord* geoms, int first, int n, WallTable& out)
{
    out.num_boxes = 0;
    for (int g = first; g < n && g < 32; ++g) {
        const GeomRecord& r = geoms[g];
        if (r.type != FF_GEOM_TRIANGLEMESH || r.bvh_root < 0) continue;
        WallTable::MeshBox& b = out.box[out.num_boxes++];
        for (int k = 0; k < 3; ++k) { b.mn[k] = r.wmin[k]; b.mx[k] = r.wmax[k]; }
        b.geom = g;
        b.pad = 0;
    }
}

int collapse_geometry_tree(const std::vector<BvhNode>& binary, std::vector<Bvh4Node>& out)
{
    out.clear();
    if (binary.empty()) return 0;
    std::vector<int> order(1, 0), index4(binary.size(), -1), level(1, 1);
    index4[0] = 0;
    auto grandchildren = [&](int n, int links[4], const float* mn[4], const float* mx[4]) {
        int slots = 0;
        const BvhNode& nd = binary[n];
        for (int side = 0; side < 2; ++side) {
            const int link = side == 0 ? nd.left : nd.right;
            if (link < 0) {
                links[slots] = link; mn[slots] = side == 0 ? nd.lmin : nd.rmin; mx[slots] = side == 0 ? nd.lmax : nd.rmax; ++slots;
            } else {
                const BvhNode& ch = binary[link];
                links[slots] = ch.left; mn[slots] = ch.lmin; mx[slots] = ch.lmax; ++slots;
                links[slots] = ch.right; mn[slots] = ch.rmin; mx[slots] = ch.rmax; ++slots;
            }
        }
        return slots;
    };
    int depth = 1;
    for (size_t i = 0; i < order.size(); ++i) {
        int links[4];
        const float *mn[4], *mx[4];
        const int slots = grandchildren(order[i], links, mn, mx);
        for (int q = 0; q < slots; ++q)
            if (links[q] >= 0) {
                index4[links[q]] = (int)order.size();
                order.push_back(links[q]);
                level.push_back(level[i] + 1);
                depth = std::max(depth, level[i] + 1);
            }
    }
    out.resize(order.size());
    for (size_t i = 0; i < order.size(); ++i) {
        int links[4];
        const float *mn[4], *mx[4];
        const int slots = grandchildren(order[i], links, mn, mx);
        Bvh4Node& o = out[i];
        for (int q = 0; q < 4; ++q) {
            for (int k = 0; k < 3; ++k) {
                o.mn[k][q] = q < slots ? mn[q][k] : std::numeric_limits<float>::infinity();
                o.mx[k][q] = q < slots ? mx[q][k] : -std::numeric_limits<float>::infinity();
            }
            o.link[q] = q >= slots ? kEmptyLink : (links[q] >= 0 ? index4[links[q]] : ~(kGeomLeafBit | ~links[q]));
        }
    }
    return depth;
}

void set_world_box(GeomRecord& r, const float omn[3], const float omx[3])
{
    using namespace ffm;
    M4 mod;
    mod.c[0] = v4(r.mod_c0[0], r.mod_c0[1], r.mod_c0[2], 0.f);
    mod.c[1] = v4(r.mod_c1[0], r.mod_c1[1], r.mod_c1[2], 0.f);
    mod.c[2] = v4(r.mod_c2[0], r.mod_c2[1], r.mod_c2[2], 0.f);
    mod.c[3] = v4(r.mod_c3[0], r.mod_c3[1], r.mod_c3[2], 1.f);
    Box wb;
    wb.reset();
    if (omn[0] <= omx[0]) {
        for (int c = 0; c < 8; ++c) {
            const V4 pw = mul(mod, v4((c & 1) ? omx[0] : omn[0], (c & 2) ? omx[1] : omn[1], (c & 4) ? omx[2] : omn[2], 1.f));
            wb.grow(&pw.x);
        }
        float big = 0.f;
        for (int k = 0; k < 3; ++k) big = std::max(big, std::max(std::fabs(wb.mn[k]), std::fabs(wb.mx[k])) + (wb.mx[k] - wb.mn[k]));
// ... 163 lines not shown

}
}

extern "C" int ff_scene_info(const FfGeometry* host_geometries, int n, FfSceneInfo* out)
{
    using namespace ff;
    clear_error();
    if (!out) return fail(FF_ERR_INVALID_ARG, "ff_scene_info: out_info is null");
    std::memset(out, 0, sizeof *out);
    CompiledScene cs;
    const BvhBuildParams bp = default_bvh_params();
    const int st = compile_scene(host_geometries, n, bp, cs);
    if (st != FF_OK) return st;
    out->num_geometries = (int)cs.geoms.size();
    for (const GeomRecord& g : cs.geoms) {
        if (g.type == FF_GEOM_TRIANGLEMESH) ++out->num_meshes;
        else ++out->num_planes;
    }
    out->bvh_nodes = (int)cs.nodes.size();
    out->bvh_max_depth = cs.max_depth;
    out->num_triangles = cs.tris.size();
    const int stack_depth = cs.max_depth + 1;
    out->lds_nodes = std::min((int)cs.nodes.size(), std::max(0, max_lds_nodes(stack_depth, 512, (int)cs.geoms.size())));
    out->lds_bytes = (int)bvh_lds_bytes(out->lds_nodes, stack_depth, 512, (int)cs.geoms.size());
    out->device_bytes = cs.geoms.size() * sizeof(GeomRecord) + cs.tris.size() * sizeof(TriRecord) + cs.nodes.size() * sizeof(BvhNode);
    int max_leaf = 0;
    out->valid = check_bvh(cs, &max_leaf) ? 1 : 0;
    out->bvh_max_leaf = max_leaf;
    double area = 0.0;
    for (const BvhNode& nd : cs.nodes) {
        const float* lo[2] = { nd.lmin, nd.rmin };
        const float* hi[2] = { nd.lmax, nd.rmax };
        for (int c = 0; c < 2; ++c) {
            const double dx = (double)hi[c][0] - lo[c][0], dy = (double)hi[c][1] - lo[c][1], dz = (double)hi[c][2] - lo[c][2];
            if (dx >= 0.0 && dy >= 0.0 && dz >= 0.0) area += dx * dy + dy * dz + dz * dx;
        }
    }
    out->bvh_child_area = (float)area;
    return FF_OK;
}

extern "C" int ff_debug_wall_table(const FfGeometry* host_geometries, int n, float* out_walls7, int max_walls)
{
    using namespace ff;
    clear_error();
    CompiledScene cs;
    const int st = compile_scene(host_geometries, n, default_bvh_params(), cs, false);
    if (st != FF_OK) return -st;
    int num_quads = 0;
    for (const GeomRecord& g : cs.geoms) num_quads += g.type == FF_GEOM_PLANE ? 1 : 0;
    WallTable t;
    build_wall_table(cs.geoms.data(), num_quads, t, std::getenv("FF_NO_WALL_PAIRS") == nullptr);
    int count = 0, i = 0;
    for (int axis = 0; axis < 3; ++axis)
        for (int k = 0; k < t.count[axis]; ++k, ++i) {
            const Wall& w = t.w[i];
            for (int side = 0; side < (w.hi_geom1 ? 2 : 1); ++side) {
                if (out_walls7 && count < max_walls) {
                    float* o = out_walls7 + (size_t)count * 7;
                    o[0] = (float)cs.geoms[side ? w.hi_geom1 - 1 : w.geom].orig_index;
                    o[1] = (float)axis;
                    o[2] = side ? w.hi_c : w.c; o[3] = w.cu; o[4] = w.hu; o[5] = w.cv; o[6] = w.hv;
                }
                ++count;
            }
        }
    return count;
}

extern "C" int ff_debug_wall_entries(const FfGeometry* host_geometries, int n)
{
    using namespace ff;
    clear_error();
    CompiledScene cs;
    const int st = compile_scene(host_geometries, n, default_bvh_params(), cs, false);
    if (st != FF_OK) return -st;
    int num_quads = 0;
    for (const GeomRecord& g : cs.geoms) num_quads += g.type == FF_GEOM_PLANE ? 1 : 0;
    WallTable t;
    build_wall_table(cs.geoms.data(), num_quads, t, std::getenv("FF_NO_WALL_PAIRS") == nullptr);
    return t.count[0] + t.count[1] + t.count[2];
}
```

### gpupathtracer_amd/csrc/ff_state.h

```cpp
#pragma once

#include <vector>

#include <hip/hip_runtime.h>

#include "ff_build.h"
#include "ff_image.h"
#include "ff_internal.h"
#include "ff_kernels.h"
#include "ff_texture.h"

struct FfDistContext;

struct FfState {
    int device = 0;
    int num_cus = 0;
    size_t device_mem_bytes = 0;
    hipStream_t stream = nullptr;
    ff::GeomRecord* d_geoms = nullptr;
    ff::TriRecord* d_tris = nullptr;
    ff::TriNormals* d_normals = nullptr;
    ff::TriUVs* d_uvs = nullptr;
    float4* d_world_normals = nullptr;
    ff::BvhNode* d_nodes = nullptr;
    ff::WallTable walls = {};
    int num_scan = 0;
    ff::Bvh4Node* d_nodes4 = nullptr;
    int num_geoms = 0, num_planes = 0, num_quads = 0, num_nodes = 0, max_depth = 0;
    int num_nodes4 = 0, max_depth4 = 0;
    int top_count = 0, top_depth = 0, top_lds_count = 0;
    int stack_entries = 1;
    int stack_lds_levels = 1;
    unsigned long long* d_cull_mask = nullptr;
    size_t cull_mask_bytes = 0;
    float4* d_primary_cache = nullptr;
    size_t primary_cache_bytes = 0;
    float4* d_start_records = nullptr;
    size_t start_records_bytes = 0;
    bool primary_has_start = false;
    int start_bounces = 0, start_shade = 0;
    struct PrimaryKey {
        float cam[24];
        int dims[12];
        unsigned pix_items;
    } primary_key = {};
    bool primary_valid = false;
    PrimaryKey last_key = {};
    bool last_key_valid = false;
    bool primary_has_mask = false;
    unsigned long long primary_culled_pixels = 0;
    bool pending_mask_reused = false, pending_mask_built = false;
    float4* d_park = nullptr;
    size_t park_bytes = 0;
    int* d_stack_spill = nullptr;
    size_t stack_spill_bytes = 0;
    bool use_pool = false;
    int scene_block_threads = 0, lds_cap = 0;
    bool has_specular = false;
    uint64_t num_tris = 0;
    bool has_scene = false;
    struct MeshSlot {
        int node_first = 0, node_count = 0, node_capacity = 0, depth = 0;
        int node4_count = 0, depth4 = 0;
        bool parents_linked = false;
    };
    int builder = FF_BUILD_HOST_SAH;
    int scene_builder = FF_BUILD_HOST_SAH;
    std::vector<ff::GeomRecord> h_geoms;
    std::vector<MeshSlot> slots;
    size_t node_capacity = 0;
    int* d_parent = nullptr;
    unsigned char* d_role = nullptr;
    FfTriangle* d_stage = nullptr;
    size_t stage_bytes = 0;
    ff::BuildScratch scratch;
    FfBuildStats build_stats = {};
    float* d_blocksums = nullptr;
    size_t blocksums_bytes = 0;
    unsigned char* d_rgb8 = nullptr;
    size_t rgb8_bytes = 0;
    float* d_radiance = nullptr;
    size_t radiance_bytes = 0;
    float4* d_tail_samples = nullptr;
    size_t tail_samples_bytes = 0;
    bool tail_forced = false;
    int tail_min_blocks = 4;
    int tail_group_spp = 8;
    float* d_accum = nullptr;
    size_t accum_bytes = 0;
    float* d_frame = nullptr;
    size_t frame_bytes = 0;
    float* d_mean = nullptr;
    size_t mean_bytes = 0;
    int accum_width = 0, accum_height = 0, accum_frames = 0;
    float4* d_gb_hits = nullptr;
    size_t gb_hits_bytes = 0;
    void* d_img_stage = nullptr;
    size_t img_stage_bytes = 0;
    float4* d_dn_work = nullptr;
    size_t dn_work_bytes = 0;
    enum { kHistoryTemporal = 0, kHistoryTaa = 1, kHistoryTaaUpscale = 2 };
    ff::ReprojectionHistory history[3];
    int taa_upscale_lo_width = 0, taa_upscale_lo_height = 0;
    float jitter_x = 0.f, jitter_y = 0.f;
    FfCameraSampling cam_sampling = { FF_PIXEL_CORNER, 0.f, 1.f, 0 };
    bool cam_active() const { return cam_sampling.pixel_filter == FF_PIXEL_BOX || cam_sampling.lens_radius > 0.f; }
    std::vector<FfGeometry> nee_geoms;
    std::vector<FfBXDF> nee_bxdfs;
    std::vector<std::vector<FfTriangle>> nee_tris;
    bool nee_valid = false;
    int nee_num_lights = 0;
    float4* d_nee_lights = nullptr;
    size_t nee_lights_bytes = 0;
    float* d_nee_pdf = nullptr;
    size_t nee_pdf_bytes = 0;
    bool env_set = false;
    bool env_sampled = false;
    int env_w = 0, env_h = 0;
    float env_rotation = 0.f;
    float4* d_env_texels = nullptr;
    size_t env_texels_bytes = 0;
    float2* d_env_alias = nullptr;
    size_t env_alias_bytes = 0;
    float* d_env_z = nullptr;
    size_t env_z_bytes = 0;
    struct Texture {
        float4* d_texels = nullptr;
        int w = 0, h = 0, flags = 0;
    };
    std::vector<Texture> textures;
    std::vector<ff::TexBinding> tex_bindings;
    int tex_bound = 0;
    ff::TexBinding* d_tex_bind = nullptr;
    size_t tex_bind_bytes = 0;
    ff::TexDesc* d_tex_desc = nullptr;
    size_t tex_desc_bytes = 0;
    std::vector<float> glossy_roughness;
    int glossy_applied = 0;
    float* d_glossy_alpha = nullptr;
    size_t glossy_alpha_bytes = 0;
    void* d_disp_const = nullptr;
    size_t disp_const_bytes = 0;
    void* d_disp_work = nullptr;
    size_t disp_work_bytes = 0;
    bool disp_has_prev = false, disp_called = false;
    float disp_prev_exposure = 0.f;
    float disp_exposure = 0.f, disp_target = 0.f;
    uint32_t disp_histogram[256] = {};
    void* d_mblur_work = nullptr;
    size_t mblur_work_bytes = 0;
    void* d_dof_work = nullptr;
    size_t dof_work_bytes = 0;
    void* d_despeckle_work = nullptr;
    size_t despeckle_work_bytes = 0;
    unsigned* d_queue = nullptr;
    unsigned long long* d_counters = nullptr;
    unsigned long long* h_counters = nullptr;
    hipEvent_t ev_begin = nullptr, ev_end = nullptr;
    bool collect_stats = false;
    struct Switches {
        bool no_last_bounce_cut = false, no_primary_cull = false, no_primary_reuse = false;
        bool no_start_records = false;
        bool no_world_normals = false;
        bool no_primary_cache = false;
        int tail_blocks = 0;
        int reuse_min_spp = 2;
        int reuse_quorum = 1;
        int queue_chunk = 0, queue_counters = 0;
        int queue_tail = -1;
        bool no_wall_table = false, no_wall_pairs = false, no_stack_spill = false, no_scan_planes = false;
        bool lds_fill = false;
        unsigned long lds_fill_words = 0, lds_fill_pattern = 0;
        int pool = -1;
        int pool_quorum = 0;
        int pool_quorum_min = 0;
        int pool_refill = 0;
        int pool_slice = 0;
        int pool_batch_min = 0;
        int lds_node_cap = -1;
        int pool_leave = -1;
        int pool_stack_levels = 0;
    } sw;
    int block_threads = ff::kBlockThreadsMax;
    bool setup_threshold_forced = false;
    int setup_threshold = 14, leaf_threshold = 20;
    FfStats stats;
    const char* last_kernel_name = nullptr;
    unsigned long long raw_counters[32] = {};
    hipGraphicsResource* pbo_resource = nullptr;
    int pbo_width = 0, pbo_height = 0;
    FfDistContext* dist = nullptr;
    int pending_launches = 0;
    uint32_t pending_flags = 0;
    unsigned pending_culled_rays_per_pixel = 0;
    bool pending = false;
    int debug_fail_alloc = -1, alloc_countdown = -1;
    int timeline_bucket_us = 0;
    unsigned* d_timeline = nullptr;
    unsigned h_timeline[1024] = {};
    std::vector<unsigned> h_timeline_rows;
};


#define FF_HIP(call)                                                                                          \
    do {                                                                                                      \
        hipError_t _e = (call);                                                                               \
        if (_e != hipSuccess) return fail(_e == hipErrorOutOfMemory ? FF_ERR_OOM : FF_ERR_HIP, "%s failed: %s (%s:%d)", #call, hipGetErrorString(_e), __FILE__, __LINE__); \
    } while (0)

namespace ff {

int ensure_bytes(void** ptr, size_t* cap, size_t need);

int check_render_call(const FfState* s, const FfCamera* camera, const FfRenderParams* params, const char* who);

int render_enqueue(FfState* s, const FfCamera* camera, const FfRenderParams* prm, int strip_rows, int part, int num_parts, int local_rows,
                   unsigned char* rgb8_dev, float* radiance_dev, int x0 = 0, int y0 = 0, int win_w = -1);
int render_finish(FfState* s);

struct PrimaryHits {
    const float4* hits;
    bool fresh;
    unsigned pix_items;
    int tiles_per_row, xlim, ylim;
};
int frame_primary_hits(FfState* s, const FfCamera* camera, const FfRenderParams* params, PrimaryHits* out);

void dist_release(FfState* s);

void nee_capture(FfState* s, const FfGeometry* g, int n, bool upload);
void nee_replace_mesh(FfState* s, int geometry_index, const FfTriangle* tris, int count);
int nee_rebuild(FfState* s);
int enqueue_nee(FfState* s, KParams& k, const FfCamera* camera, const FfRenderParams* prm, int launches, int blocks_per_launch, size_t local_pixels);
int check_camera_sampling(const FfCameraSampling* cs, const char* who);
void env_release(FfState* s);
void tex_drop_bindings(FfState* s);
int tex_sync_tables(FfState* s);
void tex_release(FfState* s);
void glossy_drop_bindings(FfState* s);
int glossy_sync_table(FfState* s);
void glossy_release(FfState* s);
void display_release(FfState* s);
void motion_blur_release(FfState* s);
void dof_release(FfState* s);
void despeckle_release(FfState* s);
int map_pbo(FfState* s, size_t need_bytes, void** out_ptr);
// ... 6 lines not shown
```

### gpupathtracer_amd/lib.py

```python
import ctypes as C
import os

import numpy as np

from . import types as T

_HERE = os.path.dirname(os.path.abspath(__file__))
LIB_PATH = os.environ.get("FF_LIB_PATH") or os.path.join(_HERE, "libfirefly_hip.so")

EXPORTS = [
    "ff_create", "ff_destroy", "ff_last_error", "ff_version", "ff_set_stream",
    "ff_geometry_init", "ff_bxdf_init", "ff_camera_init_default", "ff_camera_update_basis", "ff_camera_ray_matrix",
    "ff_render_tile", "ff_upload_scene", "ff_set_builder", "ff_update_transforms", "ff_update_mesh", "ff_build_stats", "ff_debug_download_bvh", "ff_debug_download_bvh4",
    "ff_scene_info", "ff_debug_wall_table", "ff_debug_wall_entries", "ff_render", "ff_render_strips", "ff_strips_local_rows", "ff_deinterleave_strips",
    "ff_intersect_rays", "ff_register_gl_pbo", "ff_unregister_gl_pbo", "ff_render_to_pbo",
    "ff_render_progressive", "ff_render_to_pbo_progressive", "ff_save_ppm",
    "ff_set_collect_stats", "ff_stats", "ff_debug_kernel_name", "ff_debug_counters", "ff_debug_timeline", "ff_debug_check_ieee", "ff_debug_reload_switches", "ff_load_obj", "ff_free_triangles",
    "ff_scene_file_load", "ff_scene_file_geometries", "ff_scene_file_camera", "ff_scene_file_free",
    "ff_dist_unique_id", "ff_dist_init", "ff_dist_available", "ff_dist_shutdown", "ff_dist_strip_rows", "ff_dist_strip_rows_for", "ff_dist_part_bytes", "ff_render_distributed", "ff_debug_dist_fail_rank",
    "ff_multi_create", "ff_multi_destroy", "ff_multi_count", "ff_multi_state", "ff_multi_uses_rccl", "ff_multi_upload_scene",
    "ff_multi_render", "ff_multi_render_to_pbo", "ff_multi_stats",
    "ff_gbuffer", "ff_denoise_params_init", "ff_denoise",
    "ff_temporal_params_init", "ff_denoise_temporal", "ff_temporal_reset", "ff_temporal_history",
    "ff_camera_ray_matrix_jittered", "ff_set_pixel_jitter", "ff_multi_set_pixel_jitter", "ff_jitter_sequence",
    "ff_taa_params_init", "ff_taa", "ff_taa_reset", "ff_taa_history",
    "ff_light_table", "ff_check_render_params",
    "ff_set_environment", "ff_environment_table", "ff_load_hdr", "ff_free_hdr", "ff_scene_file_environment",
    "ff_display_params_init", "ff_display", "ff_display_to_pbo", "ff_display_reset", "ff_display_state",
    "ff_srgb_thresholds", "ff_display_curve", "ff_display_exposure", "ff_save_hdr",
    "ff_texture_create", "ff_texture_destroy", "ff_set_albedo_texture", "ff_texture_sample", "ff_surface_uv",
    "ff_load_ppm", "ff_free_ppm", "ff_rgb8_to_linear", "ff_scene_file_texture_count", "ff_scene_file_texture", "ff_scene_file_albedo_map",
    "ff_set_roughness", "ff_glossy_eval", "ff_glossy_sample", "ff_scene_file_roughness",
    "ff_camera_sampling_init", "ff_set_camera_sampling", "ff_camera_sample_rays", "ff_scene_file_camera_sampling",
    "ff_upscale_params_init", "ff_upscale", "ff_upscale_host",
    "ff_taa_upscale_params_init", "ff_taa_upscale", "ff_taa_upscale_reset", "ff_taa_upscale_history",
    "ff_motion_blur_params_init", "ff_motion_blur", "ff_motion_blur_host",
    "ff_dof_params_init", "ff_dof_params_from_camera", "ff_depth_of_field", "ff_depth_of_field_host",
    "ff_despeckle_params_init", "ff_despeckle", "ff_despeckle_host",
]
DIST_ID_BYTES = 128

_lib = None


class FireflyError(RuntimeError):
    def __init__(self, status, message):
        super().__init__(f"firefly status {status}: {message}")
        self.status = status
        self.message = message


class _Tolerant:

    class _Missing:
        argtypes = restype = None

    def __init__(self, lib):
        self._lib = lib

    def __getattr__(self, name):
        try:
            return getattr(self._lib, name)
        except AttributeError:
            return _Tolerant._Missing()


def load():
    global _lib
    if _lib is not None:
        return _lib
    if not os.path.exists(LIB_PATH):
        raise ImportError(
            f"{LIB_PATH} not found: the HIP extension has not been built (run __graft_entry__.build()); "
            "there is no CPU fallback for the trace path")
    real = C.CDLL(LIB_PATH)
    lib = _Tolerant(real) if os.environ.get("FF_LIB_PATH") else real
    vp, i32, f32 = C.c_void_p, C.c_int, C.c_float
    P = C.POINTER
    lib.ff_create.argtypes = [P(vp), i32]
    lib.ff_destroy.argtypes = [vp]
    lib.ff_last_error.restype = C.c_char_p
    lib.ff_version.restype = i32
    lib.ff_set_stream.argtypes = [vp, vp]
    lib.ff_geometry_init.argtypes = [P(T.FfGeometry), i32, T.FfVec3, T.FfVec3, T.FfVec3, P(T.FfTriangle), i32, f32]
    lib.ff_geometry_init.restype = None
    lib.ff_bxdf_init.argtypes = [P(T.FfBXDF)]
    lib.ff_bxdf_init.restype = None
    lib.ff_camera_init_default.argtypes = [P(T.FfCamera), i32, i32]
    lib.ff_camera_init_default.restype = None
    lib.ff_camera_update_basis.argtypes = [P(T.FfCamera)]
    lib.ff_camera_update_basis.restype = None
    lib.ff_camera_ray_matrix.argtypes = [P(T.FfCamera), P(T.FfMat4)]
    lib.ff_camera_ray_matrix.restype = None
    lib.ff_upload_scene.argtypes = [vp, P(T.FfGeometry), i32]
    lib.ff_set_builder.argtypes = [vp, i32]
    lib.ff_update_transforms.argtypes = [vp, P(T.FfGeometry), i32]
    lib.ff_update_mesh.argtypes = [vp, i32, P(T.FfTriangle), i32, i32]
    lib.ff_build_stats.argtypes = [vp, P(T.FfBuildStats)]
    lib.ff_debug_download_bvh.argtypes = [vp, vp, i32, P(i32), vp, i32, P(i32), P(i32), i32]
    lib.ff_debug_download_bvh4.argtypes = [vp, vp, i32, P(i32), P(i32), i32]
    lib.ff_scene_info.argtypes = [P(T.FfGeometry), i32, P(T.FfSceneInfo)]
    lib.ff_debug_wall_table.argtypes = [P(T.FfGeometry), i32, P(C.c_float), i32]
    lib.ff_debug_wall_entries.argtypes = [P(T.FfGeometry), i32]
    lib.ff_render.argtypes = [vp, P(T.FfCamera), P(T.FfRenderParams), vp, i32, vp, i32]
    lib.ff_render_tile.argtypes = [vp, P(T.FfCamera), P(T.FfRenderParams), i32, i32, i32, i32, vp, i32, vp, i32]
    lib.ff_render_strips.argtypes = [vp, P(T.FfCamera), P(T.FfRenderParams), i32, i32, i32, vp, i32, vp, i32, P(i32)]
    lib.ff_strips_local_rows.argtypes = [i32, i32, i32, i32]
    lib.ff_deinterleave_strips.argtypes = [vp, vp, vp, i32, i32, i32, i32, i32]
    lib.ff_intersect_rays.argtypes = [vp, P(T.FfRay), i32, P(T.FfIntersect), i32]
    lib.ff_register_gl_pbo.argtypes = [vp, C.c_uint, i32, i32]
    lib.ff_unregister_gl_pbo.argtypes = [vp]
    lib.ff_render_to_pbo.argtypes = [vp, P(T.FfCamera), P(T.FfRenderParams)]
    lib.ff_render_progressive.argtypes = [vp, P(T.FfCamera), P(T.FfRenderParams), i32, vp, i32, vp, i32]
    lib.ff_render_to_pbo_progressive.argtypes = [vp, P(T.FfCamera), P(T.FfRenderParams), i32]
    lib.ff_save_ppm.argtypes = [C.c_char_p, vp, i32, i32]
    lib.ff_set_collect_stats.argtypes = [vp, i32]
    lib.ff_stats.argtypes = [vp, P(T.FfStats)]
    lib.ff_debug_counters.argtypes = [vp, P(C.c_ulonglong)]
    lib.ff_debug_timeline.argtypes = [vp, P(C.c_uint), P(C.c_int)]
    lib.ff_debug_kernel_name.argtypes = [vp]
    lib.ff_debug_kernel_name.restype = C.c_char_p
    lib.ff_debug_check_ieee.argtypes = [vp, P(C.c_ulonglong)]
    lib.ff_debug_reload_switches.argtypes = [vp]
    lib.ff_load_obj.argtypes = [C.c_char_p, P(P(T.FfTriangle)), P(i32)]
    lib.ff_free_triangles.argtypes = [P(T.FfTriangle)]
    lib.ff_free_triangles.restype = None
    lib.ff_scene_file_load.argtypes = [C.c_char_p, P(vp)]
    lib.ff_scene_file_geometries.argtypes = [vp, P(i32)]
    lib.ff_scene_file_geometries.restype = P(T.FfGeometry)
    lib.ff_scene_file_camera.argtypes = [vp, i32, i32, P(T.FfCamera)]
    lib.ff_scene_file_free.argtypes = [vp]
    lib.ff_scene_file_free.restype = None
    lib.ff_dist_unique_id.argtypes = [vp, i32]
    lib.ff_dist_init.argtypes = [vp, i32, i32, vp, i32]
    lib.ff_dist_shutdown.argtypes = [vp]
    lib.ff_debug_dist_fail_rank.argtypes = [vp, C.c_int]
    lib.ff_dist_available.argtypes = []
    lib.ff_dist_strip_rows.argtypes = [i32]
    lib.ff_dist_strip_rows_for.argtypes = [i32, i32]
    lib.ff_dist_part_bytes.argtypes = [i32, i32, i32, i32, i32, P(C.c_longlong)]
    lib.ff_dist_part_bytes.restype = C.c_longlong
    lib.ff_render_distributed.argtypes = [vp, P(T.FfCamera), P(T.FfRenderParams), i32, vp, i32, vp, i32]
    lib.ff_multi_create.argtypes = [P(vp), P(i32), i32]
    lib.ff_multi_destroy.argtypes = [vp]
    lib.ff_multi_count.argtypes = [vp]
    lib.ff_multi_state.argtypes = [vp, i32]
    lib.ff_multi_state.restype = vp
    lib.ff_multi_uses_rccl.argtypes = [vp]
    lib.ff_multi_upload_scene.argtypes = [vp, P(T.FfGeometry), i32]
    lib.ff_multi_render.argtypes = [vp, P(T.FfCamera), P(T.FfRenderParams), i32, vp, i32, vp, i32]
    lib.ff_multi_render_to_pbo.argtypes = [vp, P(T.FfCamera), P(T.FfRenderParams), i32]
    lib.ff_multi_stats.argtypes = [vp, P(T.FfStats)]
    lib.ff_gbuffer.argtypes = [vp, P(T.FfCamera), P(T.FfRenderParams), vp, vp, vp, vp, vp, i32]
    lib.ff_denoise_params_init.argtypes = [P(T.FfDenoiseParams)]
    lib.ff_denoise_params_init.restype = None
    lib.ff_denoise.argtypes = [vp, i32, i32, P(T.FfDenoiseParams), vp, vp, vp, vp, vp, i32, vp, i32, vp, i32]
    lib.ff_temporal_params_init.argtypes = [P(T.FfTemporalParams)]
    lib.ff_temporal_params_init.restype = None
    lib.ff_denoise_temporal.argtypes = [vp, P(T.FfCamera), i32, i32, P(T.FfTemporalParams), vp, vp, vp, vp, vp, i32, vp, i32, vp, i32]
    lib.ff_temporal_reset.argtypes = [vp]
    lib.ff_temporal_history.argtypes = [vp, vp, vp, i32]
    lib.ff_camera_ray_matrix_jittered.argtypes = [P(T.FfCamera), C.c_float, C.c_float, P(T.FfMat4)]
    lib.ff_camera_ray_matrix_jittered.restype = None
    lib.ff_set_pixel_jitter.argtypes = [vp, C.c_float, C.c_float]
    lib.ff_multi_set_pixel_jitter.argtypes = [vp, C.c_float, C.c_float]
    lib.ff_jitter_sequence.argtypes = [i32, i32, P(C.c_float), P(C.c_float)]
    lib.ff_light_table.argtypes = [P(T.FfGeometry), i32, P(T.FfLightEntry), i32, P(C.c_float)]
    lib.ff_check_render_params.argtypes = [P(T.FfRenderParams)]
    lib.ff_set_environment.argtypes = [vp, vp, i32, i32, f32, f32]
    lib.ff_environment_table.argtypes = [vp, i32, i32, vp, vp, vp, vp]
    lib.ff_load_hdr.argtypes = [C.c_char_p, P(P(C.c_float)), P(i32), P(i32)]
    lib.ff_free_hdr.argtypes = [P(C.c_float)]
    lib.ff_free_hdr.restype = None
    lib.ff_scene_file_environment.argtypes = [vp, P(C.c_char_p), P(C.c_float), P(C.c_float)]
    lib.ff_taa_params_init.argtypes = [P(T.FfTaaParams)]
    lib.ff_taa_params_init.restype = None
    lib.ff_taa.argtypes = [vp, P(T.FfCamera), i32, i32, P(T.FfTaaParams), vp, vp, vp, i32, vp, i32, vp, i32]
    lib.ff_taa_reset.argtypes = [vp]
    lib.ff_taa_history.argtypes = [vp, vp, vp, i32]
    lib.ff_display_params_init.argtypes = [P(T.FfDisplayParams)]
    lib.ff_display_params_init.restype = None
    lib.ff_display.argtypes = [vp, i32, i32, P(T.FfDisplayParams), vp, i32, vp, i32, vp, i32]
    lib.ff_display_to_pbo.argtypes = [vp, i32, i32, P(T.FfDisplayParams), vp, i32]
    lib.ff_display_reset.argtypes = [vp]
    lib.ff_display_state.argtypes = [vp, P(f32), P(f32), vp]
    lib.ff_srgb_thresholds.argtypes = [vp]
# ... 564 lines not shown
    def set_stream(self, hip_stream_ptr):
        check(self._lib.ff_set_stream(self._state, C.c_void_p(hip_stream_ptr)))

    def upload_scene(self, scene):
        check(self._lib.ff_upload_scene(self._state, scene.geometries, len(scene)))

    def set_environment(self, rgb, intensity=1.0, rotation_deg=0.0):
        a = _env_map(rgb)
        check(self._lib.ff_set_environment(self._state, a.ctypes.data, a.shape[1], a.shape[0], float(intensity), float(rotation_deg)))

    def clear_environment(self):
        check(self._lib.ff_set_environment(self._state, None, 0, 0, 0.0, 0.0))

    def create_texture(self, rgb, flags=0):
        a = _texture_image(rgb)
        tid = C.c_int(-1)
        check(self._lib.ff_texture_create(self._state, a.ctypes.data, a.shape[1], a.shape[0], int(flags), C.byref(tid)))
        return tid.value

    def destroy_texture(self, texture_id):
        check(self._lib.ff_texture_destroy(self._state, int(texture_id)))

    def set_albedo_texture(self, geometry_index, texture_id, scale=(1.0, 1.0), offset=(0.0, 0.0)):
        check(self._lib.ff_set_albedo_texture(self._state, int(geometry_index), -1 if texture_id is None else int(texture_id),
                                              float(scale[0]), float(scale[1]), float(offset[0]), float(offset[1])))

    def set_roughness(self, geometry_index, roughness):
        check(self._lib.ff_set_roughness(self._state, int(geometry_index), 0.0 if roughness is None else float(roughness)))

    def set_camera_sampling(self, sampling=None):
        check(self._lib.ff_set_camera_sampling(self._state, None if sampling is None else C.byref(sampling)))

    def apply_scene_file_materials(self, scene_file):
        for g in range(len(scene_file)):
            r = scene_file.roughness(g)
            if r is not None:
                self.set_roughness(g, r)

    def set_builder(self, builder):
        check(self._lib.ff_set_builder(self._state, builder))

    def update_transforms(self, scene):
        check(self._lib.ff_update_transforms(self._state, scene.geometries, len(scene)))

    def update_mesh(self, geometry_index, triangles, mode=T.UPDATE_REFIT):
        buf = T.triangles_from_array(triangles)
        check(self._lib.ff_update_mesh(self._state, geometry_index, buf, len(buf), mode))

    def build_stats(self):
        st = T.FfBuildStats()
        check(self._lib.ff_build_stats(self._state, C.byref(st)))
        return st

    def download_bvh(self, num_geometries):
        nn, nt = C.c_int(0), C.c_int(0)
        check(self._lib.ff_debug_download_bvh(self._state, None, 0, C.byref(nn), None, 0, C.byref(nt), None, 0))
        nodes = np.zeros(max(nn.value, 1), dtype=T.BVH_NODE_DTYPE)
        tris = np.zeros(max(nt.value, 1), dtype=T.TRI_RECORD_DTYPE)
        table = np.full((num_geometries, 5), -1, dtype=np.int32)
        check(self._lib.ff_debug_download_bvh(self._state, nodes.ctypes.data, nn.value, C.byref(nn), tris.ctypes.data, nt.value, C.byref(nt),
                                              table.ctypes.data_as(C.POINTER(C.c_int)), num_geometries))
        return nodes[:nn.value], tris[:nt.value], table

    def download_bvh4(self, num_geometries):
        cap = C.c_int(0)
        check(self._lib.ff_debug_download_bvh4(self._state, None, 0, C.byref(cap), None, 0))
        nodes = np.zeros(max(cap.value, 1), dtype=T.BVH4_NODE_DTYPE)
        table = np.full((num_geometries, 6), -1, dtype=np.int32)
        check(self._lib.ff_debug_download_bvh4(self._state, nodes.ctypes.data, cap.value, C.byref(cap),
                                               table.ctypes.data_as(C.POINTER(C.c_int)), num_geometries))
        return nodes[:cap.value], table

    def set_collect_stats(self, on):
        check(self._lib.ff_set_collect_stats(self._state, 1 if on else 0))

    def stats(self):
        st = T.FfStats()
        check(self._lib.ff_stats(self._state, C.byref(st)))
        return st

    def kernel_name(self):
        return self._lib.ff_debug_kernel_name(self._state).decode()

    def check_ieee(self):
        buf = (C.c_ulonglong * 2)()
        check(self._lib.ff_debug_check_ieee(self._state, buf))
        return int(buf[0]), int(buf[1])

    def reload_switches(self):
        check(self._lib.ff_debug_reload_switches(self._state))

    def debug_counters(self):
        buf = (C.c_ulonglong * 32)()
        check(self._lib.ff_debug_counters(self._state, buf))
        return list(buf)

    def debug_timeline(self):
        buf = (C.c_uint * 1024)()
        us = C.c_int(0)
        check(self._lib.ff_debug_timeline(self._state, buf, C.byref(us)))
        return int(us.value), np.frombuffer(buf, dtype=np.uint32).copy()

    def render(self, camera, params, want_rgb8=True, want_radiance=True):
        h, w = params.height, params.width
        rgb8 = np.zeros((h, w, 3), dtype=np.uint8) if want_rgb8 else None
        rad = np.zeros((h, w, 3), dtype=np.float32) if want_radiance else None
        check(self._lib.ff_render(self._state, C.byref(camera), C.byref(params),
                                  rgb8.ctypes.data if want_rgb8 else None, 0,
                                  rad.ctypes.data if want_radiance else None, 0))
        return rgb8, rad

    def render_progressive(self, camera, params, frame_index):
        h, w = params.height, params.width
        rgb8 = np.zeros((h, w, 3), dtype=np.uint8)
        rad = np.zeros((h, w, 3), dtype=np.float32)
        check(self._lib.ff_render_progressive(self._state, C.byref(camera), C.byref(params), frame_index, rgb8.ctypes.data, 0, rad.ctypes.data, 0))
        return rgb8, rad

    def render_tile(self, camera, params, x0, y0, w, h):
        rgb8 = np.zeros((h, w, 3), dtype=np.uint8)
        rad = np.zeros((h, w, 3), dtype=np.float32)
        check(self._lib.ff_render_tile(self._state, C.byref(camera), C.byref(params), x0, y0, w, h, rgb8.ctypes.data, 0, rad.ctypes.data, 0))
        return rgb8, rad

    def render_device(self, camera, params, rgb8_ptr=None, radiance_ptr=None):
        check(self._lib.ff_render(self._state, C.byref(camera), C.byref(params),
                                  C.c_void_p(rgb8_ptr) if rgb8_ptr else None, 1,
                                  C.c_void_p(radiance_ptr) if radiance_ptr else None, 1))

    def gbuffer(self, camera, params):
        h, w = params.height, params.width
        out = {name: np.zeros((h, w) + shape, dtype=dt) for name, dt, shape in GBUFFER_CHANNELS}
        check(self._lib.ff_gbuffer(self._state, C.byref(camera), C.byref(params), *(out[name].ctypes.data for name, _, _ in GBUFFER_CHANNELS), 0))
        return out

    def gbuffer_device(self, camera, params, depth_ptr=None, position_ptr=None, normal_ptr=None, albedo_ptr=None, ids_ptr=None):
        ptrs = [C.c_void_p(p) if p else None for p in (depth_ptr, position_ptr, normal_ptr, albedo_ptr, ids_ptr)]
        check(self._lib.ff_gbuffer(self._state, C.byref(camera), C.byref(params), *ptrs, 1))

    def denoise(self, radiance, gbuffer, dn=None):
        rad = np.ascontiguousarray(radiance, dtype=np.float32)
        h, w = rad.shape[:2]
        dn = dn if dn is not None else denoise_params()
        g = {k: np.ascontiguousarray(gbuffer[k], dtype=np.int32 if k == "ids" else np.float32) for k in ("position", "normal", "albedo", "ids")}
        rgb8 = np.zeros((h, w, 3), dtype=np.uint8)
        out = np.zeros((h, w, 3), dtype=np.float32)
        check(self._lib.ff_denoise(self._state, w, h, C.byref(dn), rad.ctypes.data, g["position"].ctypes.data, g["normal"].ctypes.data,
                                   g["albedo"].ctypes.data, g["ids"].ctypes.data, 0, rgb8.ctypes.data, 0, out.ctypes.data, 0))
        return rgb8, out

    def denoise_device(self, width, height, radiance_ptr, position_ptr, normal_ptr, albedo_ptr, ids_ptr, dn=None, rgb8_ptr=None, radiance_out_ptr=None):
        dn = dn if dn is not None else denoise_params()
        vp = lambda p: C.c_void_p(p) if p else None
        check(self._lib.ff_denoise(self._state, width, height, C.byref(dn), vp(radiance_ptr), vp(position_ptr), vp(normal_ptr), vp(albedo_ptr),
                                   vp(ids_ptr), 1, vp(rgb8_ptr), 1, vp(radiance_out_ptr), 1))

    def denoise_temporal(self, radiance, gbuffer, camera, tp=None):
        rad = np.ascontiguousarray(radiance, dtype=np.float32)
        h, w = rad.shape[:2]
        if rad.shape != (h, w, 3) or any(np.shape(gbuffer[k])[:2] != (h, w) for k in ("position", "normal", "albedo", "ids")):
            raise ValueError("denoise_temporal: radiance must be [H,W,3] and the G-buffer of the same size")
        tp = tp if tp is not None else temporal_params()
        g = {k: np.ascontiguousarray(gbuffer[k], dtype=np.int32 if k == "ids" else np.float32) for k in ("position", "normal", "albedo", "ids")}
        rgb8 = np.zeros((h, w, 3), dtype=np.uint8)
        out = np.zeros((h, w, 3), dtype=np.float32)
        check(self._lib.ff_denoise_temporal(self._state, C.byref(camera), w, h, C.byref(tp), rad.ctypes.data, g["position"].ctypes.data,
# ... 340 lines not shown
```

### include/firefly/ff_api.h

```cpp
#ifndef FIREFLY_FF_API_H
#define FIREFLY_FF_API_H

#include "ff_types.h"

#ifdef __cplusplus
extern "C" {
#endif

#if defined(_WIN32)
#define FF_API __declspec(dllexport)
#else
#define FF_API __attribute__((visibility("default")))
#endif

typedef enum FfStatus {
    FF_OK                 = 0,
    FF_ERR_INVALID_ARG    = 1,
    FF_ERR_NO_DEVICE      = 2,
    FF_ERR_HIP            = 3,
    FF_ERR_NO_SCENE       = 4,
    FF_ERR_UNSUPPORTED    = 5,
    FF_ERR_GL_UNAVAILABLE = 6,
    FF_ERR_IO             = 7,
    FF_ERR_OOM            = 8,
    FF_ERR_COMM           = 9
} FfStatus;

typedef struct FfState FfState;


FF_API int ff_create(FfState** out_state, int device_id);
FF_API int ff_destroy(FfState* state);

FF_API const char* ff_last_error(void);

FF_API int ff_version(void);

FF_API int ff_set_stream(FfState* state, void* hip_stream);


FF_API void ff_geometry_init(FfGeometry* g, int geometry_type, FfVec3 position, FfVec3 rotation_deg,
                             FfVec3 scale, FfTriangle* triangles, int number_of_triangles, float radius);

FF_API void ff_bxdf_init(FfBXDF* b);

FF_API void ff_camera_init_default(FfCamera* c, int width, int height);

FF_API void ff_camera_update_basis(FfCamera* c);

FF_API void ff_camera_ray_matrix(const FfCamera* c, FfMat4* out_inv_view_times_inv_proj);

FF_API void ff_camera_ray_matrix_jittered(const FfCamera* c, float jx, float jy, FfMat4* out);

FF_API int ff_set_pixel_jitter(FfState* state, float jx, float jy);

FF_API int ff_jitter_sequence(int index, int period, float* jx, float* jy);


FF_API int ff_upload_scene(FfState* state, const FfGeometry* host_geometries, int n);


FF_API int ff_set_builder(FfState* state, int builder);

FF_API int ff_update_transforms(FfState* state, const FfGeometry* host_geometries, int n);

FF_API int ff_update_mesh(FfState* state, int geometry_index, const FfTriangle* triangles, int count, int mode);

FF_API int ff_build_stats(FfState* state, FfBuildStats* out_stats);

FF_API int ff_debug_download_bvh(FfState* state, void* nodes, int max_nodes, int* out_nodes, void* tris, int max_tris, int* out_tris,
                                 int* mesh_table, int max_geometries);

FF_API int ff_debug_download_bvh4(FfState* state, void* nodes4, int max_nodes, int* out_capacity, int* mesh_table, int max_geometries);

FF_API int ff_scene_info(const FfGeometry* host_geometries, int n, FfSceneInfo* out_info);

FF_API int ff_debug_wall_table(const FfGeometry* host_geometries, int n, float* out_walls7, int max_walls);
FF_API int ff_debug_wall_entries(const FfGeometry* host_geometries, int n);


FF_API int ff_render(FfState* state, const FfCamera* camera, const FfRenderParams* params,
                     void* rgb8, int rgb8_on_device, float* radiance, int radiance_on_device);

FF_API int ff_render_strips(FfState* state, const FfCamera* camera, const FfRenderParams* params,
                            int strip_rows, int part, int num_parts,
                            void* rgb8, int rgb8_on_device, float* radiance, int radiance_on_device,
                            int* out_local_rows);

FF_API int ff_render_tile(FfState* state, const FfCamera* camera, const FfRenderParams* params, int x0, int y0, int w, int h, void* rgb8,
                          int rgb8_on_device, float* radiance, int radiance_on_device);

FF_API int ff_strips_local_rows(int height, int strip_rows, int part, int num_parts);

FF_API int ff_deinterleave_strips(FfState* state, const void* src_dev, void* dst_dev, int width, int height,
                                  int strip_rows, int num_parts, int elem_bytes);


#define FF_DIST_ID_BYTES 128
FF_API int ff_dist_unique_id(void* out_id, int bytes);
FF_API int ff_dist_init(FfState* state, int rank, int world_size, const void* id, int bytes);
FF_API int ff_dist_available(void);
FF_API int ff_dist_shutdown(FfState* state);

FF_API int ff_dist_strip_rows_for(int height, int world_size);
FF_API int ff_dist_strip_rows(int world_size);

FF_API long long ff_dist_part_bytes(int width, int height, int strip_rows, int part, int num_parts, long long* out_offset);

FF_API int ff_render_distributed(FfState* state, const FfCamera* camera, const FfRenderParams* params, int strip_rows,
                                 void* rgb8, int rgb8_on_device, float* radiance, int radiance_on_device);
FF_API int ff_debug_dist_fail_rank(FfState* state, int rank);

typedef struct FfMulti FfMulti;
FF_API int ff_multi_create(FfMulti** out_multi, const int* device_ids, int n);
FF_API int ff_multi_destroy(FfMulti* multi);
FF_API int ff_multi_count(const FfMulti* multi);
FF_API FfState* ff_multi_state(FfMulti* multi, int index);
FF_API int ff_multi_uses_rccl(const FfMulti* multi);
FF_API int ff_multi_upload_scene(FfMulti* multi, const FfGeometry* host_geometries, int n);
FF_API int ff_multi_render(FfMulti* multi, const FfCamera* camera, const FfRenderParams* params, int strip_rows,
                           void* rgb8, int rgb8_on_device, float* radiance, int radiance_on_device);
FF_API int ff_multi_render_to_pbo(FfMulti* multi, const FfCamera* camera, const FfRenderParams* params, int strip_rows);
FF_API int ff_multi_stats(FfMulti* multi, FfStats* out);
FF_API int ff_multi_set_pixel_jitter(FfMulti* multi, float jx, float jy);

FF_API int ff_intersect_rays(FfState* state, const FfRay* rays, int n, FfIntersect* out, int trace_mode);


FF_API int ff_register_gl_pbo(FfState* state, unsigned int pbo, int width, int height);
FF_API int ff_unregister_gl_pbo(FfState* state);

FF_API int ff_render_to_pbo(FfState* state, const FfCamera* camera, const FfRenderParams* params);


FF_API int ff_render_progressive(FfState* state, const FfCamera* camera, const FfRenderParams* params, int frame_index, void* rgb8, int rgb8_on_device,
                                 float* radiance, int radiance_on_device);

FF_API int ff_render_to_pbo_progressive(FfState* state, const FfCamera* camera, const FfRenderParams* params, int frame_index);



FF_API int ff_light_table(const FfGeometry* host_geometries, int n, FfLightEntry* out_entries, int max_entries, float* out_pdf_area);

FF_API int ff_check_render_params(const FfRenderParams* params);



FF_API int ff_set_environment(FfState* state, const float* rgb, int width, int height, float intensity, float rotation_deg);

FF_API int ff_environment_table(const float* rgb, int width, int height, float* out_probability, float* out_alias_probability, int* out_alias,
                                float* out_pdf);

FF_API int ff_load_hdr(const char* path, float** out_rgb, int* out_width, int* out_height);
FF_API void ff_free_hdr(float* rgb);



FF_API int ff_texture_create(FfState* state, const float* rgb, int width, int height, int flags, int* out_id);

FF_API int ff_texture_destroy(FfState* state, int id);

// ... 182 lines not shown
```

Baseline: 15560 Mrays/s.

## Replace enclosing Cornell box walls with a single room-exit slab test

At scene setup the host looks for an axis-aligned box formed by full-size walls (the room) and removes those walls from the per-ray wall table. The trace kernel gets a ROOM template variant that computes the exit face of the room with one slab test and accepts it as the hit only when a conservative in-box and steepness check passes. Otherwise the ray falls back to the slow path for those geometries. This is meant to cut the per-ray cost of screening the six enclosing planes, at the cost of more kernel instantiations and a larger kernel parameter block.

```diff
diff --git a/gpupathtracer_amd/csrc/ff_api.cpp b/gpupathtracer_amd/csrc/ff_api.cpp
--- a/gpupathtracer_amd/csrc/ff_api.cpp
+++ b/gpupathtracer_amd/csrc/ff_api.cpp
@@ -178,6 +178,12 @@
     }
     build_wall_table(s->h_geoms.data(), s->sw.no_wall_table ? 0 : (s->num_geoms > kChunkGeometries ? s->num_scan : s->num_quads), s->walls, !s->sw.no_wall_pairs);
     if (s->num_geoms <= kChunkGeometries) add_mesh_boxes(s->h_geoms.data(), s->num_planes, s->num_geoms, s->walls);
+    if (s->num_geoms <= kChunkGeometries) {
+        extract_room(s->walls, s->room, s->walls_rest);
+    } else {
+        s->room = Room();
+        s->walls_rest = s->walls;
+    }
     s->stack_entries = depth4 + 1 + (s->top_depth > 0 ? s->top_depth + 1 : 0);
     if (!s->setup_threshold_forced) {
         int biggest = 1;
@@ -336,6 +342,7 @@
     k.top_lds_count = s->top_lds_count;
     k.num_scan = s->num_scan;
     k.walls = s->walls;
+    k.room = s->room;
 }
 
 int attach_stack_spill(FfState* s, KParams& k, int grid, int block_threads)
@@ -641,6 +648,8 @@
         s->start_bounces = bounces;
         s->start_shade = prm->shade_mode;
     }
+    const bool room_pays = !s->sw.no_room && s->lds_cap >= s->num_nodes4;
+    bool room_used = false;
     for (int l = 0; l < launches; ++l) {
         k.block_begin = l * blocks_per_launch;
         k.block_end = std::min(num_blocks, (l + 1) * blocks_per_launch);
@@ -655,8 +664,10 @@
         }
         if (l > 0) FF_HIP(hipMemsetAsync(s->d_queue, 0, (size_t)k.queue_counters * kQueueStride * sizeof(unsigned), st));
         FF_HIP(launch_trace(k, prm->trace_mode, s->collect_stats, grid, block_threads, st, &s->last_kernel_name, pool, false, use_start,
-                            !s->sw.no_world_normals));
-    }
+                            !s->sw.no_world_normals, room_pays ? &s->walls_rest : nullptr, &room_used));
+    }
+    s->last_room_faces = 0;
+    for (int f = 0; room_used && f < 6; ++f) s->last_room_faces += s->room.geom[f] >= 0 ? 1 : 0;
     FF_HIP(launch_combine(k, st));
     FF_HIP(hipEventRecord(s->ev_end, st));
     FF_HIP(hipMemcpyAsync(s->h_counters, s->d_counters, kCounterWords * sizeof(unsigned long long), hipMemcpyDeviceToHost, st));
@@ -765,6 +776,7 @@
     w.no_primary_cache = std::getenv("FF_NO_PRIMARY_CACHE") != nullptr;
     w.no_start_records = std::getenv("FF_NO_START_RECORDS") != nullptr;
     w.no_world_normals = std::getenv("FF_NO_WORLD_NORMALS") != nullptr;
+    w.no_room = std::getenv("FF_NO_ROOM") != nullptr;
     if (const char* e = std::getenv("FF_TAIL_BLOCKS")) w.tail_blocks = std::max(1, std::min(3, std::atoi(e)));
     if (const char* e = std::getenv("FF_REUSE_MIN_SPP")) w.reuse_min_spp = std::max(1, std::atoi(e));
     if (const char* e = std::getenv("FF_REUSE_QUORUM")) w.reuse_quorum = std::max(1, std::min(65, std::atoi(e)));
@@ -1764,6 +1776,8 @@
 
 const char* ff_debug_kernel_name(FfState* s) { return s && s->last_kernel_name ? s->last_kernel_name : ""; }
 
+int ff_debug_room_faces(FfState* s) { return s ? s->last_room_faces : 0; }
+
 int ff_stats(FfState* s, FfStats* out)
 {
     clear_error();
diff --git a/gpupathtracer_amd/csrc/ff_internal.h b/gpupathtracer_amd/csrc/ff_internal.h
--- a/gpupathtracer_amd/csrc/ff_internal.h
+++ b/gpupathtracer_amd/csrc/ff_internal.h
@@ -96,6 +96,15 @@
     } box[32];
 };
 
+struct Room {
+    float cc[3], hh[3];
+    float lo[3], hi[3];
+    int geom[6];
+    unsigned mask;
+    int pad;
+};
+bool extract_room(const WallTable& table, Room& room, WallTable& rest);
+
 void build_wall_table(const struct GeomRecord* geoms, int limit, WallTable& out, bool pairing = true);
 void add_mesh_boxes(const struct GeomRecord* geoms, int first, int n, WallTable& out);
 
diff --git a/gpupathtracer_amd/csrc/ff_k_traverse.h b/gpupathtracer_amd/csrc/ff_k_traverse.h
--- a/gpupathtracer_amd/csrc/ff_k_traverse.h
+++ b/gpupathtracer_amd/csrc/ff_k_traverse.h
@@ -226,12 +226,38 @@
     best_g = nearer ? g : best_g;
 }
 
-template <bool STATS>
-__device__ __forceinline__ void screen_walls(const WallTable& W, const Ray& wr, const WorldSlab& ws, float wlen, Segment& S, unsigned& slow, Counters& cnt)
+__device__ __forceinline__ void room_exit(const Room& R, const Ray& wr, const WorldSlab& ws, float wlen, float D, float th, float ax, float ay, float az,
+                                          float aix, float aiy, float aiz, float gmin, float& best_d, int& best_g, unsigned& slow)
+{
+    const bool in = wr.ox - R.lo[0] > th && R.hi[0] - wr.ox > th && wr.oy - R.lo[1] > th && R.hi[1] - wr.oy > th && wr.oz - R.lo[2] > th && R.hi[2] - wr.oz > th;
+    const bool upx = ws.ix > 0.0f, upy = ws.iy > 0.0f, upz = ws.iz > 0.0f;
+    const float tx = __builtin_fmaf(upx ? R.hi[0] : R.lo[0], ws.ix, ws.ox);
+    const float ty = __builtin_fmaf(upy ? R.hi[1] : R.lo[1], ws.iy, ws.oy);
+    const float tz = __builtin_fmaf(upz ? R.hi[2] : R.lo[2], ws.iz, ws.oz);
+    const float t = fminf(tx, fminf(ty, tz));
+    const bool kx = t == tx, ky = t == ty;
+    const float px = __builtin_fmaf(t, wr.dx, wr.ox), py = __builtin_fmaf(t, wr.dy, wr.oy), pz = __builtin_fmaf(t, wr.dz, wr.oz);
+    const float ex = fabsf(px - R.cc[0]) - R.hh[0], ey = fabsf(py - R.cc[1]) - R.hh[1], ez = fabsf(pz - R.cc[2]) - R.hh[2];
+    const float m = kx ? fmaxf(ey, ez) : (ky ? fmaxf(ez, ex) : fmaxf(ex, ey));
+    const float ai = kx ? aix : (ky ? aiy : aiz);
+    const float au = kx ? fmaxf(ay, az) : (ky ? fmaxf(az, ax) : fmaxf(ax, ay));
+    const float dl = D * __builtin_fmaf(au, ai, 1.0f), tt = th * ai;
+    const int g = kx ? (upx ? R.geom[1] : R.geom[0]) : (ky ? (upy ? R.geom[3] : R.geom[2]) : (upz ? R.geom[5] : R.geom[4]));
+    const bool steep = (kx ? ax : (ky ? ay : az)) >= gmin;
+    const bool sure = in && m <= -dl && t > tt && steep;
+    slow |= sure ? 0u : R.mask;
+    const bool hit = sure && g >= 0;
+    best_d = hit ? t * wlen : best_d;
+    best_g = hit ? g : best_g;
+}
+
+template <bool STATS, bool ROOM = false>
+__device__ __forceinline__ void screen_walls(const WallTable& W, const Ray& wr, const WorldSlab& ws, float wlen, Segment& S, unsigned& slow, Counters& cnt,
+                                             const Room* room = nullptr)
 {
     const int nx = W.count[0], ny = nx + W.count[1], nz = ny + W.count[2];
-    if (nz == 0) return;
-    if (STATS) { cnt.planes += (unsigned)nz; probe_round(cnt.wall_rounds); }
+    if (!ROOM && nz == 0) return;
+    if (STATS) { cnt.planes += (unsigned)nz + (ROOM ? 1u : 0u); probe_round(cnt.wall_rounds); }
     const float D = 2.0e-5f * ((fabsf(wr.ox) + fabsf(wr.oy)) + (fabsf(wr.oz) + W.margin_s));
     const float th = 0.05f * D;
     const float ax = fabsf(wr.dx), ay = fabsf(wr.dy), az = fabsf(wr.dz);
@@ -240,6 +266,7 @@
     float best_d = kInf;
     int best_g = -1;
     bool tie = false;
+    if constexpr (ROOM) room_exit(*room, wr, ws, wlen, D, th, ax, ay, az, aix, aiy, aiz, gmin, best_d, best_g, slow);
     Wall cur = W.w[0];
     int i = 0;
     {
@@ -286,9 +313,10 @@
     return (S.pend.geom >= 0 ? 1u << (S.pend.geom & 31) : 0u) | (S.best.geom >= 0 ? 1u << (S.best.geom & 31) : 0u);
 }
 
-template <bool STATS, class LDS>
+template <bool STATS, bool ROOM = false, class LDS>
 __device__ __forceinline__ bool scan_records(const LDS& L, const WallTable& W, const GeomRecord* __restrict__ geoms, int num_geoms, int num_planes,
-                                           const TriRecord* __restrict__ tris, const Ray& wr, Segment& S, Counters& cnt, bool cut, unsigned emitters)
+                                           const TriRecord* __restrict__ tris, const Ray& wr, Segment& S, Counters& cnt, bool cut, unsigned emitters,
+                                           const Room* room = nullptr)
 {
     const int prim_end = num_planes;
     const float wlen = __builtin_amdgcn_rcpf(inv_length(wr));
@@ -297,7 +325,8 @@
     if (STATS) tb0 = __builtin_amdgcn_s_memtime();
     const WorldSlab ws = make_world_slab(wr);
     unsigned quads = 0u;
-    screen_walls<STATS>(W, wr, ws, wlen, S, quads, cnt);
+    if constexpr (ROOM) screen_walls<STATS, true>(W, wr, ws, wlen, S, quads, cnt, room);
+    else screen_walls<STATS>(W, wr, ws, wlen, S, quads, cnt);
     for (int g = 0; g < prim_end; ++g) {
         if ((W.mask >> g) & 1u) continue;
         const float4 bmin = lds_geom4(L, g, 14), bmax = lds_geom4(L, g, 15);
@@ -358,11 +387,12 @@
     }
 }
 
-template <bool STATS, class LDS>
+template <bool STATS, bool ROOM = false, class LDS>
 __device__ __forceinline__ bool begin_segment(const LDS& L, const WallTable& W, const GeomRecord* __restrict__ geoms, int num_geoms, int num_planes,
                                               const TriRecord* __restrict__ tris, const Ray& wr, Segment& S, Counters& cnt, bool cut = false,
-                                              unsigned emitters = 0u)
-{
+                                              unsigned emitters = 0u, const Room* room = nullptr)
+{
+    static_assert(!ROOM || !LDS::big, "room exit: scenes that scan their records only");
     S.best.dist = kInf;
     S.best.geom = -1;
     S.best.rec = -1;
@@ -383,7 +413,8 @@
         S.cur = 0;
         return false;
     }
-    return scan_records<STATS>(L, W, geoms, num_geoms, num_planes, tris, wr, S, cnt, cut, emitters);
+    if constexpr (ROOM) return scan_records<STATS, true>(L, W, geoms, num_geoms, num_planes, tris, wr, S, cnt, cut, emitters, room);
+    else return scan_records<STATS>(L, W, geoms, num_geoms, num_planes, tris, wr, S, cnt, cut, emitters);
 }
 
 __device__ __forceinline__ void refresh_tbound(Segment& S)
diff --git a/gpupathtracer_amd/csrc/ff_kernels.h b/gpupathtracer_amd/csrc/ff_kernels.h
--- a/gpupathtracer_amd/csrc/ff_kernels.h
+++ b/gpupathtracer_amd/csrc/ff_kernels.h
@@ -75,6 +75,7 @@
     int start_bounces;
     const float4* tri_world_normals;
     const float4* geom_world_normals;
+    Room room;
 };
 constexpr int kRaySlots = 30, kRaySlotFirst = 2, kRaySlotStride = 16;
 constexpr int kAnsweredWord = kRaySlotStride * kRaySlotFirst + 1;
@@ -140,7 +141,8 @@
 size_t pool_lds_bytes(int block_threads);
 
 hipError_t launch_trace(const KParams& p, int trace_mode, bool collect_stats, int grid_blocks, int block_threads, hipStream_t stream,
-                        const char** kernel_name = nullptr, bool pool = false, bool prepass = false, bool start = false, bool world_normals = false);
+                        const char** kernel_name = nullptr, bool pool = false, bool prepass = false, bool start = false, bool world_normals = false,
+                        const WallTable* room_rest = nullptr, bool* room_used = nullptr);
 hipError_t launch_world_normals(const GeomRecord* geoms, const TriRecord* tris, int num_geoms, int max_tri_count, float4* tri_out, float4* geom_out,
                                 hipStream_t stream);
 hipError_t launch_combine(const KParams& p, hipStream_t stream);
diff --git a/gpupathtracer_amd/csrc/ff_kernels.hip b/gpupathtracer_amd/csrc/ff_kernels.hip
--- a/gpupathtracer_amd/csrc/ff_kernels.hip
+++ b/gpupathtracer_amd/csrc/ff_kernels.hip
@@ -5,11 +5,12 @@
 namespace {
 
 
-template <bool STATS, int BLOCK, bool EXTRAS, int BIG = 0, bool PREPASS = false, bool START = false, bool WN = false>
+template <bool STATS, int BLOCK, bool EXTRAS, int BIG = 0, bool PREPASS = false, bool START = false, bool WN = false, bool ROOM = false>
 __global__ __launch_bounds__(BLOCK) void trace_bvh_kernel(const KParams p)
 {
     static_assert(!START || (!EXTRAS && BIG == 0 && !PREPASS), "start records: the diffuse small-scene kernel only");
     static_assert(!WN || (!EXTRAS && BIG == 0 && !PREPASS), "normal tables: the diffuse small-scene kernels only");
+    static_assert(!ROOM || WN, "room exit: the kernels on the normal tables only");
     const int tid = threadIdx.x;
     const int lane = tid & (kWave - 1);
     const LdsT<BIG> L = make_lds<BIG>(p.lds_nodes, p.stack_depth, BLOCK, tid, EXTRAS ? p.num_quads : 0x7fffffff, EXTRAS ? p.trinormals : nullptr,
@@ -180,7 +181,10 @@
         bool over = false;
         if (setup && active && !(P.b == 0 && reuse)) {
             if (STATS) probe_round(cnt.segment_rounds);
-            over = begin_segment<STATS>(L, p.walls, p.geoms, p.num_geoms, p.num_planes, p.tris, P.ray, S, cnt, p.cut_last != 0 && P.b == p.bounces - 1, p.emitter_mask);
+            if constexpr (ROOM)
+                over = begin_segment<STATS, true>(L, p.walls, p.geoms, p.num_geoms, p.num_planes, p.tris, P.ray, S, cnt, p.cut_last != 0 && P.b == p.bounces - 1, p.emitter_mask, &p.room);
+            else
+                over = begin_segment<STATS>(L, p.walls, p.geoms, p.num_geoms, p.num_planes, p.tris, P.ray, S, cnt, p.cut_last != 0 && P.b == p.bounces - 1, p.emitter_mask);
             cnt.rays += 1;
             inflight = true;
         }
@@ -892,14 +896,16 @@
 }
 
 
-#define FF_TRACE_BVH_KERNELS_OF(X, B)                                                                                                                \
-    X(false, B, false, 0, false, false, false) X(true, B, false, 0, false, false, false) X(false, B, true, 0, false, false, false)                   \
-    X(true, B, true, 0, false, false, false) X(false, B, true, 1, false, false, false) X(true, B, true, 1, false, false, false)                      \
-    X(false, B, true, 2, false, false, false) X(true, B, true, 2, false, false, false)                                                               \
-    X(false, B, true, 0, true, false, false) X(false, B, true, 1, true, false, false) X(false, B, true, 2, true, false, false)                       \
-    X(false, B, false, 0, false, true, false) X(true, B, false, 0, false, true, false)                                                               \
-    X(false, B, false, 0, false, false, true) X(true, B, false, 0, false, false, true)                                                               \
-    X(false, B, false, 0, false, true, true) X(true, B, false, 0, false, true, true)
+#define FF_TRACE_BVH_KERNELS_OF(X, B)                                                                                                                                       \
+    X(false, B, false, 0, false, false, false, false) X(true, B, false, 0, false, false, false, false) X(false, B, true, 0, false, false, false, false)                     \
+    X(true, B, true, 0, false, false, false, false) X(false, B, true, 1, false, false, false, false) X(true, B, true, 1, false, false, false, false)                        \
+    X(false, B, true, 2, false, false, false, false) X(true, B, true, 2, false, false, false, false)                                                                        \
+    X(false, B, true, 0, true, false, false, false) X(false, B, true, 1, true, false, false, false) X(false, B, true, 2, true, false, false, false)                         \
+    X(false, B, false, 0, false, true, false, false) X(true, B, false, 0, false, true, false, false)                                                                        \
+    X(false, B, false, 0, false, false, true, false) X(true, B, false, 0, false, false, true, false)                                                                        \
+    X(false, B, false, 0, false, true, true, false) X(true, B, false, 0, false, true, true, false)                                                                          \
+    X(false, B, false, 0, false, false, true, true) X(true, B, false, 0, false, false, true, true)                                                                          \
+    X(false, B, false, 0, false, true, true, true) X(true, B, false, 0, false, true, true, true)
 #define FF_TRACE_BVH_KERNELS(X) FF_TRACE_BVH_KERNELS_OF(X, 512) FF_TRACE_BVH_KERNELS_OF(X, 768) FF_TRACE_BVH_KERNELS_OF(X, 1024)
 #define FF_NAME_START_false ""
 #define FF_NAME_START_true ", true"
@@ -922,8 +928,8 @@
 hipError_t prepare_kernels()
 {
     hipError_t e;
-#define FF_X(STATS, B, EXTRAS, BIG, PREPASS, START, WN) \
-    if ((e = allow_full_lds(&trace_bvh_kernel<STATS, B, EXTRAS, BIG, PREPASS, START, WN>)) != hipSuccess) return e;
+#define FF_X(STATS, B, EXTRAS, BIG, PREPASS, START, WN, ROOM) \
+    if ((e = allow_full_lds(&trace_bvh_kernel<STATS, B, EXTRAS, BIG, PREPASS, START, WN, ROOM>)) != hipSuccess) return e;
     FF_TRACE_BVH_KERNELS(FF_X)
 #undef FF_X
 #define FF_X(STATS, B, EXTRAS) \
@@ -961,8 +967,9 @@
 }
 
 hipError_t launch_trace(const KParams& p, int trace_mode, bool collect_stats, int grid_blocks, int block_threads, hipStream_t stream,
-                        const char** kernel_name, bool pool, bool prepass, bool start, bool world_normals)
-{
+                        const char** kernel_name, bool pool, bool prepass, bool start, bool world_normals, const WallTable* room_rest, bool* room_used)
+{
+    if (room_used) *room_used = false;
     const dim3 grid(grid_blocks);
     const char* name = "";
     if (!prepass && trace_mode == FF_TRACE_BVH && pool && p.num_geoms <= kChunkGeometries && block_threads == 1024)
@@ -975,9 +982,17 @@
         const int threads = block_threads == 1024 ? 1024 : (block_threads == 768 ? 768 : 512);
         const bool stats = !prepass && collect_stats, extras = prepass || big != 0 || needs_extras(p), from_start = !prepass && start;
         const bool wn = world_normals && !extras && p.shade_mode == FF_SHADE_DIFFUSE_PATH && p.tri_world_normals != nullptr && p.geom_world_normals != nullptr;
-#define FF_X(STATS, B, EXTRAS, BIG, PREPASS, START, WN)                                                                                              \
-    if (stats == STATS && threads == B && extras == EXTRAS && big == BIG && prepass == PREPASS && from_start == START && wn == WN) {                 \
-        hipLaunchKernelGGL((trace_bvh_kernel<STATS, B, EXTRAS, BIG, PREPASS, START, WN>), grid, block, lds, stream, p);                              \
+        const bool room = wn && room_rest != nullptr && p.room.mask != 0u;
+        KParams with_rest;
+        if (room) {
+            with_rest = p;
+            with_rest.walls = *room_rest;
+        }
+        const KParams& pl = room ? with_rest : p;
+        if (room && room_used) *room_used = true;
+#define FF_X(STATS, B, EXTRAS, BIG, PREPASS, START, WN, ROOM)                                                                                        \
+    if (stats == STATS && threads == B && extras == EXTRAS && big == BIG && prepass == PREPASS && from_start == START && wn == WN && room == ROOM) { \
+        hipLaunchKernelGGL((trace_bvh_kernel<STATS, B, EXTRAS, BIG, PREPASS, START, WN, ROOM>), grid, block, lds, stream, pl);                       \
         name = "trace_bvh_kernel<" #STATS ", " #B ", " #EXTRAS ", " #BIG ", " #PREPASS FF_NAME_START_##START ">";                                    \
     } else
         FF_TRACE_BVH_KERNELS(FF_X) return hipErrorInvalidValue;
diff --git a/gpupathtracer_amd/csrc/ff_scene.cpp b/gpupathtracer_amd/csrc/ff_scene.cpp
--- a/gpupathtracer_amd/csrc/ff_scene.cpp
+++ b/gpupathtracer_amd/csrc/ff_scene.cpp
@@ -707,6 +707,96 @@
     if (ratio > 1.f) {
         out.margin_s += (ratio - 1.f) * 3.f * scale_s;
     }
+}
+
+bool extract_room(const WallTable& table, Room& room, WallTable& rest)
+{
+    std::memset(&room, 0, sizeof room);
+    rest = table;
+    struct Flat {
+        int axis;
+        float c, cu, hu, cv, hv;
+        int geom;
+    };
+    std::vector<Flat> walls;
+    {
+        int i = 0;
+        for (int axis = 0; axis < 3; ++axis)
+            for (int k = 0; k < table.count[axis]; ++k, ++i) {
+                const Wall& w = table.w[i];
+                walls.push_back({ axis, w.c, w.cu, w.hu, w.cv, w.hv, w.geom });
+                if (w.hi_geom1) walls.push_back({ axis, w.hi_c, w.cu, w.hu, w.cv, w.hv, w.hi_geom1 - 1 });
+            }
+    }
+    auto same = [](float c0, float h0, float c1, float h1) {
+        const float tol = 1.0e-6f * (std::fabs(c0) + std::fabs(h0));
+        return std::fabs(c0 - c1) <= tol && std::fabs(h0 - h1) <= tol;
+    };
+    for (size_t a = 0; a < walls.size(); ++a)
+        for (size_t b = a + 1; b < walls.size(); ++b) {
+            const Flat &A = walls[a], &B = walls[b];
+            if (A.axis == B.axis) continue;
+            float cc[3], hh[3];
+            bool have[3] = { false, false, false }, ok = true;
+            for (const Flat* f : { &A, &B }) {
+                const int uv[2] = { (f->axis + 1) % 3, (f->axis + 2) % 3 };
+                const float c2[2] = { f->cu, f->cv }, h2[2] = { f->hu, f->hv };
+                for (int j = 0; j < 2; ++j) {
+                    if (have[uv[j]]) {
+                        if (!same(cc[uv[j]], hh[uv[j]], c2[j], h2[j])) ok = false;
+                        continue;
+                    }
+                    cc[uv[j]] = c2[j];
+                    hh[uv[j]] = h2[j];
+                    have[uv[j]] = true;
+                }
+            }
+            if (!ok || !(hh[0] > 0.f && hh[1] > 0.f && hh[2] > 0.f)) continue;
+            float hmin[3] = { hh[0], hh[1], hh[2] };
+            Room r;
+            std::memset(&r, 0, sizeof r);
+            for (int k = 0; k < 6; ++k) r.geom[k] = -1;
+            int faces = 0;
+            for (const Flat& f : walls) {
+                const int k = f.axis, u = (k + 1) % 3, v = (k + 2) % 3;
+                const float tol = 1.0e-6f * (std::fabs(cc[k]) + hh[k]);
+                int side = -1;
+                if (std::fabs(f.c - (cc[k] - hh[k])) <= tol) side = 0;
+                else if (std::fabs(f.c - (cc[k] + hh[k])) <= tol) side = 1;
+                if (side < 0) continue;
+                const bool whole = same(cc[u], hh[u], f.cu, f.hu) && same(cc[v], hh[v], f.cv, f.hv);
+                if (!whole || r.geom[2 * k + side] >= 0) { ok = false; break; }
+                hmin[u] = std::min(hmin[u], f.hu);
+                hmin[v] = std::min(hmin[v], f.hv);
+                r.geom[2 * k + side] = f.geom;
+                (side ? r.hi : r.lo)[k] = f.c;
+                r.mask |= 1u << f.geom;
+                ++faces;
+            }
+            if (!ok || faces < 3) continue;
+            for (int k = 0; k < 3; ++k) {
+                r.cc[k] = cc[k];
+                r.hh[k] = hmin[k];
+                if (r.geom[2 * k] < 0) r.lo[k] = cc[k] - hh[k];
+                if (r.geom[2 * k + 1] < 0) r.hi[k] = cc[k] + hh[k];
+            }
+            room = r;
+            std::memset(rest.count, 0, sizeof rest.count);
+            std::memset(rest.w, 0, sizeof rest.w);
+            int n = 0, i = 0;
+            for (int axis = 0; axis < 3; ++axis)
+                for (int k = 0; k < table.count[axis]; ++k, ++i) {
+                    Wall w = table.w[i];
+                    const bool lo_out = (r.mask >> w.geom) & 1u, hi_out = w.hi_geom1 && ((r.mask >> (w.hi_geom1 - 1)) & 1u);
+                    if (lo_out && (hi_out || !w.hi_geom1)) continue;
+                    if (lo_out) { w.c = w.hi_c; w.geom = w.hi_geom1 - 1; }
+                    if (lo_out || hi_out) { w.hi_geom1 = 0; w.hi_c = 0.f; }
+                    rest.w[n++] = w;
+                    rest.count[axis] += 1;
+                }
+            return true;
+        }
+    return false;
 }
 
 void add_mesh_boxes(const GeomRecord* geoms, int first, int n, WallTable& out)
@@ -1036,3 +1126,27 @@
     build_wall_table(cs.geoms.data(), num_quads, t, std::getenv("FF_NO_WALL_PAIRS") == nullptr);
     return t.count[0] + t.count[1] + t.count[2];
 }
+
+extern "C" int ff_debug_room(const FfGeometry* host_geometries, int n, float* out_room13)
+{
+    using namespace ff;
+    clear_error();
+    CompiledScene cs;
+    const int st = compile_scene(host_geometries, n, default_bvh_params(), cs, false);
+    if (st != FF_OK) return -st;
+    int num_quads = 0;
+    for (const GeomRecord& g : cs.geoms) num_quads += g.type == FF_GEOM_PLANE ? 1 : 0;
+    WallTable t, rest;
+    build_wall_table(cs.geoms.data(), n > 32 ? 0 : num_quads, t, std::getenv("FF_NO_WALL_PAIRS") == nullptr);
+    Room r;
+    extract_room(t, r, rest);
+    int faces = 0, left = 0;
+    for (int k = 0; k < 6; ++k) faces += r.geom[k] >= 0 && r.mask ? 1 : 0;
+    for (int i = 0; i < rest.count[0] + rest.count[1] + rest.count[2]; ++i) left += rest.w[i].hi_geom1 ? 2 : 1;
+    if (out_room13) {
+        for (int k = 0; k < 3; ++k) { out_room13[k] = faces ? r.lo[k] : 0.f; out_room13[3 + k] = faces ? r.hi[k] : 0.f; }
+        for (int k = 0; k < 6; ++k) out_room13[6 + k] = faces && r.geom[k] >= 0 ? (float)cs.geoms[r.geom[k]].orig_index : -1.f;
+        out_room13[12] = (float)left;
+    }
+    return faces;
+}
diff --git a/gpupathtracer_amd/csrc/ff_state.h b/gpupathtracer_amd/csrc/ff_state.h
--- a/gpupathtracer_amd/csrc/ff_state.h
+++ b/gpupathtracer_amd/csrc/ff_state.h
@@ -24,6 +24,9 @@
     float4* d_world_normals = nullptr;
     ff::BvhNode* d_nodes = nullptr;
     ff::WallTable walls = {};
+    ff::Room room = {};
+    ff::WallTable walls_rest = {};
+    int last_room_faces = 0;
     int num_scan = 0;
     ff::Bvh4Node* d_nodes4 = nullptr;
     int num_geoms = 0, num_planes = 0, num_quads = 0, num_nodes = 0, max_depth = 0;
@@ -162,6 +165,7 @@
         bool no_last_bounce_cut = false, no_primary_cull = false, no_primary_reuse = false;
         bool no_start_records = false;
         bool no_world_normals = false;
+        bool no_room = false;
         bool no_primary_cache = false;
         int tail_blocks = 0;
         int reuse_min_spp = 2;
diff --git a/gpupathtracer_amd/lib.py b/gpupathtracer_amd/lib.py
--- a/gpupathtracer_amd/lib.py
+++ b/gpupathtracer_amd/lib.py
@@ -12,7 +12,7 @@
     "ff_create", "ff_destroy", "ff_last_error", "ff_version", "ff_set_stream",
     "ff_geometry_init", "ff_bxdf_init", "ff_camera_init_default", "ff_camera_update_basis", "ff_camera_ray_matrix",
     "ff_render_tile", "ff_upload_scene", "ff_set_builder", "ff_update_transforms", "ff_update_mesh", "ff_build_stats", "ff_debug_download_bvh", "ff_debug_download_bvh4",
-    "ff_scene_info", "ff_debug_wall_table", "ff_debug_wall_entries", "ff_render", "ff_render_strips", "ff_strips_local_rows", "ff_deinterleave_strips",
+    "ff_scene_info", "ff_debug_wall_table", "ff_debug_wall_entries", "ff_debug_room", "ff_debug_room_faces", "ff_render", "ff_render_strips", "ff_strips_local_rows", "ff_deinterleave_strips",
     "ff_intersect_rays", "ff_register_gl_pbo", "ff_unregister_gl_pbo", "ff_render_to_pbo",
     "ff_render_progressive", "ff_render_to_pbo_progressive", "ff_save_ppm",
     "ff_set_collect_stats", "ff_stats", "ff_debug_kernel_name", "ff_debug_counters", "ff_debug_timeline", "ff_debug_check_ieee", "ff_debug_reload_switches", "ff_load_obj", "ff_free_triangles",
@@ -102,6 +102,8 @@
     lib.ff_scene_info.argtypes = [P(T.FfGeometry), i32, P(T.FfSceneInfo)]
     lib.ff_debug_wall_table.argtypes = [P(T.FfGeometry), i32, P(C.c_float), i32]
     lib.ff_debug_wall_entries.argtypes = [P(T.FfGeometry), i32]
+    lib.ff_debug_room.argtypes = [P(T.FfGeometry), i32, P(C.c_float)]
+    lib.ff_debug_room_faces.argtypes = [vp]
     lib.ff_render.argtypes = [vp, P(T.FfCamera), P(T.FfRenderParams), vp, i32, vp, i32]
     lib.ff_render_tile.argtypes = [vp, P(T.FfCamera), P(T.FfRenderParams), i32, i32, i32, i32, vp, i32, vp, i32]
     lib.ff_render_strips.argtypes = [vp, P(T.FfCamera), P(T.FfRenderParams), i32, i32, i32, vp, i32, vp, i32, P(i32)]
@@ -832,6 +834,9 @@
     def kernel_name(self):
         return self._lib.ff_debug_kernel_name(self._state).decode()
 
+    def room_faces(self):
+        return int(self._lib.ff_debug_room_faces(self._state))
+
     def check_ieee(self):
         buf = (C.c_ulonglong * 2)()
         check(self._lib.ff_debug_check_ieee(self._state, buf))
diff --git a/include/firefly/ff_api.h b/include/firefly/ff_api.h
--- a/include/firefly/ff_api.h
+++ b/include/firefly/ff_api.h
@@ -77,6 +77,8 @@
 
 FF_API int ff_debug_wall_table(const FfGeometry* host_geometries, int n, float* out_walls7, int max_walls);
 FF_API int ff_debug_wall_entries(const FfGeometry* host_geometries, int n);
+FF_API int ff_debug_room(const FfGeometry* host_geometries, int n, float* out_room13);
+FF_API int ff_debug_room_faces(FfState* state);
 
 
 FF_API int ff_render(FfState* state, const FfCamera* camera, const FfRenderParams* params,
```

Result: no change. 15700 Mrays/s, median of 6 (+0.9%).
